# SnowCheetos/CassMantle

Hardware: AMD Instinct MI355X
Metric: SD-1.5 512^2 50-step images/sec (whole node) + p50 guess-score latency (higher is better)
Workload: dtype bf16; 1 GPU; model=sd15 UNet/VAE/CLIP (512x512, 50 steps pndm, cfg 7.5), global_batch=4, seq_len=4096, parallelism=dp1 (rooms)

## Files before the change

### cassmantle_amd/models/layers.py

```python
from __future__ import annotations

import math
import os
from typing import Optional

import torch
import torch.nn as nn

from .. import ops


def _param(shape, std, gen: Optional[torch.Generator], dtype) -> nn.Parameter:
    t = torch.randn(*shape, generator=gen, dtype=torch.float32) * std
    return nn.Parameter(t.to(dtype), requires_grad=False)


def _zeros(shape, dtype) -> nn.Parameter:
    return nn.Parameter(torch.zeros(*shape, dtype=dtype), requires_grad=False)


def _ones(shape, dtype) -> nn.Parameter:
    return nn.Parameter(torch.ones(*shape, dtype=dtype), requires_grad=False)


_GN_FUSE = os.environ.get("CASSMANTLE_GN_FUSE", "1") != "0"
_UP2 = os.environ.get("CASSMANTLE_UP2", "1") != "0"


class StatsArena:

    def __init__(self) -> None:
        self._bufs: dict = {}
        self._need: dict = {}
        self.key = None
        self.buf: Optional[torch.Tensor] = None
        self.off = 0
        self.on = False

    def begin(self, key, x: torch.Tensor) -> "StatsArena":
        self.on = x.device.type == "cuda" and ops.get_mode() == "hip" and _GN_FUSE
        self.key, self.off = key, 0
        if not self.on:
            return self
        self.buf = self._bufs.get(key)
        need = self._need.get(key, 0)
        if need and self.buf is None:
            self.buf = self._bufs[key] = torch.empty(need, device=x.device, dtype=torch.int64)
        if self.buf is not None:
            ops.zero_(self.buf)
        self.device = x.device
        return self

    def take_rows(self, rows: int) -> Optional[torch.Tensor]:
        s = self.take(1, rows)
        return None if s is None else s.view(rows, 2)

    def take(self, B: int, C: int) -> Optional[torch.Tensor]:
        if not self.on:
            return None
        n = B * C * 2
        end = self.off + n
        if self.buf is not None and end <= self.buf.numel():
            s = self.buf[self.off:end].view(B, C, 2)
        else:
            self._need[self.key] = max(self._need.get(self.key, 0), end)
            s = ops.new_stats(B, C, self.device)
        self.off = end
        return s


class Linear(nn.Module):
    def __init__(self, fin: int, fout: int, bias: bool = True, gen=None, dtype=torch.bfloat16,
                 std: Optional[float] = None):
        super().__init__()
        self.fin, self.fout = fin, fout
        self.weight = _param((fout, fin), std if std is not None else 1.0 / math.sqrt(fin), gen, dtype)
        self.bias = _param((fout,), 0.02, gen, dtype) if bias else None

    def forward(self, x, residual=None, act=None, stats=None, row_stats=None):
        return ops.linear(x, self.weight, self.bias, residual=residual, act=act, stats=stats, row_stats=row_stats)


class Conv2d(nn.Module):

    def __init__(self, cin: int, cout: int, k: int = 3, stride: int = 1, padding: Optional[int] = None,
                 bias: bool = True, gen=None, dtype=torch.bfloat16):
        super().__init__()
        self.cin, self.cout, self.k, self.stride = cin, cout, k, stride
        self.padding = (k // 2) if padding is None else padding
        self.weight = _param((cout, k, k, cin), 1.0 / math.sqrt(cin * k * k), gen, dtype)
        self.bias = _param((cout,), 0.02, gen, dtype) if bias else None

    upsampling = False
    pad_in = 0

    def _derived(self, name: str, key, fn):
        buf = self._buffers.get(name)
        if buf is None or getattr(self, "_key_" + name, None) != key or buf.device != self.weight.device:
            self.register_buffer(name, fn(), persistent=False)
            setattr(self, "_key_" + name, key)
        return self._buffers[name]

    def up2_weights(self):
        return self._derived("w4", self.weight._version, lambda: ops.fold_upsample_weights(self.weight))

    def padded_weight(self, cin: int):
        return self._derived("wpad", (self.weight._version, cin),
                             lambda: torch.nn.functional.pad(self.weight, (0, cin - self.cin)).contiguous())

    def prepare(self) -> None:
        if self.upsampling and self.k == 3 and self.cin % 64 == 0:
            self.up2_weights()
        if self.pad_in > self.cin:
            self.padded_weight(self.pad_in)

    def forward(self, x, residual=None, upsample=False, chan_bias=None, stats=None, out=None):
        if out is not None:
            w = self.padded_weight(x.shape[-1]) if x.shape[-1] > self.cin else self.weight
            return ops.conv2d(x, w, self.bias, self.stride, self.padding, residual=residual,
                              upsample=upsample, chan_bias=chan_bias, stats=stats, out=out)
        if x.shape[-1] > self.cin:
            return ops.conv2d(x, self.padded_weight(x.shape[-1]), self.bias, self.stride, self.padding,
                              residual=residual, upsample=upsample, chan_bias=chan_bias, stats=stats)
        if upsample and self.k == 3 and self.stride == 1 and _UP2 and x.device.type == "cuda" \
                and ops.get_mode() == "hip" and self.cin % 64 == 0:
            return ops.conv2d_up2(x, self.weight, self.up2_weights(), self.bias, residual=residual,
                                  chan_bias=chan_bias, stats=stats)
        if self.k == 1 and self.stride == 1 and not upsample and chan_bias is None:
            return ops.linear(x, self.weight.view(self.cout, self.cin), self.bias, residual=residual, stats=stats)
        return ops.conv2d(x, self.weight, self.bias, self.stride, self.padding, residual=residual,
                          upsample=upsample, chan_bias=chan_bias, stats=stats)


class GroupNorm(nn.Module):
    def __init__(self, groups: int, channels: int, eps: float = 1e-5, dtype=torch.bfloat16):
        super().__init__()
        self.groups, self.eps = groups, eps
        self.weight = _ones((channels,), dtype)
        self.bias = _zeros((channels,), dtype)

    def forward(self, x, silu=False, stats=None, stats2=None):
        return ops.group_norm(x, self.groups, self.weight, self.bias, self.eps, silu, stats=stats, stats2=stats2)


class LayerNorm(nn.Module):
    def __init__(self, dim: int, eps: float = 1e-5, dtype=torch.bfloat16):
        super().__init__()
        self.eps = eps
        self.weight = _ones((dim,), dtype)
        self.bias = _zeros((dim,), dtype)

    def forward(self, x):
        return ops.layer_norm(x, self.weight, self.bias, self.eps)


class SelfAttention(nn.Module):

    def __init__(self, dim: int, heads: int, gen=None, dtype=torch.bfloat16, qkv_bias=False,
                 out_bias=True):
        super().__init__()
        self.dim, self.heads = dim, heads
        self.head_dim = dim // heads
        self.to_qkv = Linear(dim, 3 * dim, bias=qkv_bias, gen=gen, dtype=dtype)
        self.to_out = Linear(dim, dim, bias=out_bias, gen=gen, dtype=dtype)

    def forward(self, x, residual=None, causal=False, kv_lens=None, fp8=False, qkv=None, kv8=None,
                row_stats=None):
        if qkv is None:
            qkv = self.to_qkv(x)
        B, N = qkv.shape[0], qkv.shape[1]
        C = self.dim
        qkv = qkv.view(B, N, 3, self.heads, self.head_dim)
        if kv8 is not None:
            assert fp8 and kv_lens is None, "kv8: fp8 self-attention without key lengths"
            o = ops.attention(qkv[:, :, 0], qkv[:, :, 1], qkv[:, :, 2], causal=causal, fp8=True, kv8=kv8)
        else:
            o = ops.attention(qkv[:, :, 0], qkv[:, :, 1], qkv[:, :, 2], causal=causal, kv_lens=kv_lens, fp8=fp8)
        return self.to_out(o.reshape(B, N, C), residual=residual, row_stats=row_stats)


class CrossAttention(nn.Module):
    def __init__(self, dim: int, ctx_dim: int, heads: int, gen=None, dtype=torch.bfloat16):
        super().__init__()
        self.dim, self.heads = dim, heads
        self.head_dim = dim // heads
        self.to_q = Linear(dim, dim, bias=False, gen=gen, dtype=dtype)
        self.to_kv = Linear(ctx_dim, 2 * dim, bias=False, gen=gen, dtype=dtype)
        self.to_out = Linear(dim, dim, bias=True, gen=gen, dtype=dtype)

    _kv = None
    _kv8 = None

    def forward(self, x, ctx, residual=None, fp8=False, q=None, row_stats=None):
        if q is None:
            q = self.to_q(x)
        B, N = q.shape[0], q.shape[1]
        C = self.dim
        q = q.view(B, N, self.heads, self.head_dim)
        kv8 = None
        if self._kv is not None and self._kv.shape[0] == B:
            kv = self._kv.view(B, self._kv.shape[1], 2, self.heads, self.head_dim)
            kv8 = self._kv8 if fp8 else None
        else:
            kv = self.to_kv(ctx).view(B, ctx.shape[1], 2, self.heads, self.head_dim)
        o = ops.attention(q, kv[:, :, 0], kv[:, :, 1], fp8=fp8, kv8=kv8)
        return self.to_out(o.reshape(B, N, C), residual=residual, row_stats=row_stats)


class GEGLUFeedForward(nn.Module):
    def __init__(self, dim: int, mult: int = 4, gen=None, dtype=torch.bfloat16):
        super().__init__()
        inner = dim * mult
        self.proj_in = Linear(dim, 2 * inner, gen=gen, dtype=dtype)
        self.proj_out = Linear(inner, dim, gen=gen, dtype=dtype)

    def forward(self, x, residual=None):
        return self.proj_out(self.proj_in(x, act="geglu"), residual=residual)
```

### cassmantle_amd/models/unet.py

```python
from __future__ import annotations

import os
from dataclasses import dataclass, field
from typing import List, Optional, Sequence, Tuple

import torch
import torch.nn as nn

from .. import ops
from .layers import (Conv2d, CrossAttention, GEGLUFeedForward, GroupNorm, LayerNorm, Linear,
                     SelfAttention, StatsArena)


@dataclass
class UNetConfig:
    in_channels: int = 4
    out_channels: int = 4
    block_out_channels: Tuple[int, ...] = (320, 640, 1280, 1280)
    down_attn: Tuple[bool, ...] = (True, True, True, False)
    transformer_depth: Tuple[int, ...] = (1, 1, 1, 1)
    mid_transformer_depth: int = 1
    layers_per_block: int = 2
    heads: Tuple[int, ...] = (8, 8, 8, 8)
    head_dim: Optional[int] = None
    cross_attention_dim: int = 768
    norm_groups: int = 32
    norm_eps: float = 1e-5
    transformer_norm_eps: float = 1e-6
    time_proj_dim: int = 320
    time_embed_dim: int = 1280
    linear_projection: bool = False
    addition_embed: bool = False
    addition_time_embed_dim: int = 256
    projection_class_embeddings_input_dim: int = 2816
    sample_size: int = 64

    def level_heads(self, i: int) -> int:
        if self.head_dim is not None:
            return self.block_out_channels[i] // self.head_dim
        return self.heads[i]


SD15_UNET = UNetConfig()
SDXL_UNET = UNetConfig(block_out_channels=(320, 640, 1280), down_attn=(False, True, True),
                       transformer_depth=(0, 2, 10), mid_transformer_depth=10, heads=(5, 10, 20),
                       head_dim=64, cross_attention_dim=2048, linear_projection=True,
                       addition_embed=True, sample_size=128)
TINY_UNET = UNetConfig(block_out_channels=(32, 64), down_attn=(True, False), transformer_depth=(1, 1),
                       heads=(2, 2), layers_per_block=1, cross_attention_dim=32, norm_groups=8,
                       time_proj_dim=32, time_embed_dim=64, sample_size=8)


class ResnetBlock(nn.Module):
    def __init__(self, cin: int, cout: int, temb: int, groups: int, eps: float, gen, dtype):
        super().__init__()
        self.norm1 = GroupNorm(groups, cin, eps, dtype)
        self.conv1 = Conv2d(cin, cout, 3, gen=gen, dtype=dtype)
        self.time_emb_proj = Linear(temb, cout, gen=gen, dtype=dtype)
        self.norm2 = GroupNorm(groups, cout, eps, dtype)
        self.conv2 = Conv2d(cout, cout, 3, gen=gen, dtype=dtype)
        self.conv_shortcut = Conv2d(cin, cout, 1, padding=0, gen=gen, dtype=dtype) if cin != cout else None

    def forward(self, x, temb_silu, tb_all=None, arena: Optional[StatsArena] = None, xs=None, xs2=None):
        pair = isinstance(x, tuple)
        B = x[0].shape[0] if pair else x.shape[0]
        cout = self.conv1.cout
        if pair:
            g = self.norm1
            h = ops.group_norm_cat(x[0], x[1], g.groups, g.weight, g.bias, g.eps, True, stats=xs, stats2=xs2)
        else:
            h = self.norm1(x, silu=True, stats=xs, stats2=xs2)
        if tb_all is not None:
            tb = tb_all[:, self._tb_off:self._tb_off + self.time_emb_proj.fout]
        else:
            tb = self.time_emb_proj(temb_silu)
        s1 = arena.take(B, cout) if arena is not None else None
        h = self.conv1(h, chan_bias=tb, stats=s1)
        h = self.norm2(h, silu=True, stats=s1)
        if pair and self.conv_shortcut is None:
            sc = torch.cat(x, dim=-1)
        elif pair:
            cs = self.conv_shortcut
            sc = ops.linear_cat(x[0], x[1], cs.weight.view(cs.cout, cs.cin), cs.bias)
        else:
            sc = self.conv_shortcut(x) if self.conv_shortcut is not None else x
        s2 = arena.take(B, cout) if arena is not None else None
        return self.conv2(h, residual=sc, stats=s2), s2


_LN_FOLD = os.environ.get("CASSMANTLE_LN_FOLD", "1") == "1"
_LN_ROWSTATS = os.environ.get("CASSMANTLE_LN_ROWSTATS", "1") == "1"
_GN_FOLD = os.environ.get("CASSMANTLE_GN_FOLD", "1") == "1"
_FF_ROWSTATS = os.environ.get("CASSMANTLE_FF_ROWSTATS", "1") == "1"


def _row_stats_wanted(x: torch.Tensor) -> bool:
    return (_LN_ROWSTATS and x.device.type == "cuda" and ops.get_mode() == "hip" and ops.LN_FOLD_MODE == 1
            and x.shape[-1] not in (320, 640) and x.shape[-1] % 8 == 0 and x.numel() // x.shape[-1] >= 1024)


_FP8_KV_EPILOGUE = os.environ.get("CASSMANTLE_FP8_KV_EPILOGUE", "1") == "1"


class BasicTransformerBlock(nn.Module):
    def __init__(self, dim: int, heads: int, ctx_dim: int, gen, dtype):
        super().__init__()
        self.norm1 = LayerNorm(dim, 1e-5, dtype)
        self.attn1 = SelfAttention(dim, heads, gen=gen, dtype=dtype)
        self.norm2 = LayerNorm(dim, 1e-5, dtype)
        self.attn2 = CrossAttention(dim, ctx_dim, heads, gen=gen, dtype=dtype)
        self.norm3 = LayerNorm(dim, 1e-5, dtype)
        self.ff = GEGLUFeedForward(dim, 4, gen=gen, dtype=dtype)

    _folds = None

    def _fold_sources(self):
        return ((self.norm1, self.attn1.to_qkv), (self.norm2, self.attn2.to_q), (self.norm3, self.ff.proj_in))

    def folds(self):
        key = tuple((n.weight._version, None if n.bias is None else n.bias._version, l.weight._version,
                     None if l.bias is None else l.bias._version) for n, l in self._fold_sources())
        buf = self._buffers.get("fold0_w")
        if buf is None or self._fold_key != key or buf.device != self.norm1.weight.device:
            for i, (n, l) in enumerate(self._fold_sources()):
                for tag, t in zip(("w", "s", "b"), ops.ln_fold(n.weight, n.bias, l.weight, l.bias)):
                    self.register_buffer(f"fold{i}_{tag}", t, persistent=False)
            self._fold_key = key
        return tuple((self._buffers[f"fold{i}_w"], self._buffers[f"fold{i}_s"], self._buffers[f"fold{i}_b"])
                     for i in range(3))

    def forward(self, x, ctx, fp8=False, arena: Optional[StatsArena] = None, xrs=None, out_stats=False):
        if _LN_FOLD and x.device.type == "cuda" and ops.get_mode() == "hip":
            f = self.folds()
            n1, n2, n3 = self.norm1, self.norm2, self.norm3
            want = arena is not None and _row_stats_wanted(x)
            rows = x.numel() // x.shape[-1]
            kv8 = None
            if fp8 and _FP8_KV_EPILOGUE and ops.kv8_ok(x, self.attn1.head_dim):
                kv8 = ops.kv8_image(x.shape[0], x.shape[1], x.shape[2], x.device)
            qkv = ops.ln_linear(x, n1.weight, n1.bias, n1.eps, self.attn1.to_qkv.weight, fold=f[0], kv8=kv8,
                                row_stats=xrs if want else None)
            r2 = arena.take_rows(rows) if want else None
            x = self.attn1(None, residual=x, fp8=fp8, qkv=qkv, kv8=kv8, row_stats=r2)
            q = ops.ln_linear(x, n2.weight, n2.bias, n2.eps, self.attn2.to_q.weight, fold=f[1], row_stats=r2)
            r3 = arena.take_rows(rows) if want else None
            x = self.attn2(None, ctx, residual=x, fp8=fp8, q=q, row_stats=r3)
            h = ops.ln_linear(x, n3.weight, n3.bias, n3.eps, self.ff.proj_in.weight, act="geglu", fold=f[2],
                              row_stats=r3)
            r4 = arena.take_rows(rows) if (want and out_stats and _FF_ROWSTATS) else None
            return self.ff.proj_out(h, residual=x, row_stats=r4), r4
        x = self.attn1(self.norm1(x), residual=x, fp8=fp8)
        x = self.attn2(self.norm2(x), ctx, residual=x, fp8=fp8)
        x = self.ff(self.norm3(x), residual=x)
        return x, None


class Transformer2D(nn.Module):
    def __init__(self, dim: int, heads: int, depth: int, ctx_dim: int, groups: int, gen, dtype):
        super().__init__()
        self.norm = GroupNorm(groups, dim, 1e-6, dtype)
        self.proj_in = Linear(dim, dim, gen=gen, dtype=dtype)
        self.transformer_blocks = nn.ModuleList(
            [BasicTransformerBlock(dim, heads, ctx_dim, gen, dtype) for _ in range(depth)])
        self.proj_out = Linear(dim, dim, gen=gen, dtype=dtype)

    def forward(self, x, ctx, fp8=False, arena: Optional[StatsArena] = None, xs=None):
        B, H, W, C = x.shape
        hrs = None
        if (_GN_FOLD and xs is not None and C == 320 and (H * W) % 256 == 0 and x.device.type == "cuda"
                and ops.get_mode() == "hip"):
            n = self.norm
            h = ops.gn_linear(x.view(B, H * W, C), xs, n.weight, n.bias, n.groups, n.eps, self.proj_in.weight,
                              self.proj_in.bias)
        else:
            h = self.norm(x, stats=xs).view(B, H * W, C)
            hrs = arena.take_rows(B * H * W) if (arena is not None and _LN_FOLD and _row_stats_wanted(h)) else None
            h = self.proj_in(h, row_stats=hrs)
        rs = hrs
        nblk = len(self.transformer_blocks)
        for i, blk in enumerate(self.transformer_blocks):
            h, rs = blk(h, ctx, fp8=fp8, arena=arena, xrs=rs, out_stats=i + 1 < nblk)
        so = arena.take(B, C) if arena is not None else None
        return self.proj_out(h, residual=x.view(B, H * W, C), stats=so).view(B, H, W, C), so


class Downsample(nn.Module):
    def __init__(self, c: int, gen, dtype):
        super().__init__()
        self.conv = Conv2d(c, c, 3, stride=2, padding=1, gen=gen, dtype=dtype)

    def forward(self, x, arena: Optional[StatsArena] = None):
        so = arena.take(x.shape[0], self.conv.cout) if arena is not None else None
        return self.conv(x, stats=so), so


class Upsample(nn.Module):
    def __init__(self, c: int, gen, dtype):
        super().__init__()
        self.conv = Conv2d(c, c, 3, gen=gen, dtype=dtype)
        self.conv.upsampling = True

    def forward(self, x, arena: Optional[StatsArena] = None):
        so = arena.take(x.shape[0], self.conv.cout) if arena is not None else None
        return self.conv(x, upsample=True, stats=so), so


class UNet(nn.Module):
    def __init__(self, cfg: UNetConfig = SD15_UNET, seed: int = 0, dtype=torch.bfloat16):
        super().__init__()
        self.cfg = cfg
        gen = torch.Generator().manual_seed(seed)
        ch = cfg.block_out_channels
        g, eps, te = cfg.norm_groups, cfg.norm_eps, cfg.time_embed_dim
        self.conv_in = Conv2d(cfg.in_channels, ch[0], 3, gen=gen, dtype=dtype)
        self.conv_in.pad_in = 8 if cfg.in_channels % 8 else 0
        self.time_linear_1 = Linear(cfg.time_proj_dim, te, gen=gen, dtype=dtype)
        self.time_linear_2 = Linear(te, te, gen=gen, dtype=dtype)
        if cfg.addition_embed:
            self.add_linear_1 = Linear(cfg.projection_class_embeddings_input_dim, te, gen=gen, dtype=dtype)
            self.add_linear_2 = Linear(te, te, gen=gen, dtype=dtype)
        self.down = nn.ModuleList()
        skip_ch: List[int] = [ch[0]]
        cur = ch[0]
        n = len(ch)
        for i in range(n):
            blk = nn.Module()
            blk.resnets = nn.ModuleList()
            blk.attentions = nn.ModuleList()
            for j in range(cfg.layers_per_block):
                blk.resnets.append(ResnetBlock(cur, ch[i], te, g, eps, gen, dtype))
                cur = ch[i]
                if cfg.down_attn[i]:
                    blk.attentions.append(Transformer2D(cur, cfg.level_heads(i), cfg.transformer_depth[i],
                                                       cfg.cross_attention_dim, g, gen, dtype))
                skip_ch.append(cur)
            blk.downsampler = Downsample(cur, gen, dtype) if i < n - 1 else None
            if i < n - 1:
                skip_ch.append(cur)
            self.down.append(blk)
        self.mid_res1 = ResnetBlock(cur, cur, te, g, eps, gen, dtype)
        self.mid_attn = Transformer2D(cur, cfg.level_heads(n - 1), cfg.mid_transformer_depth,
                                      cfg.cross_attention_dim, g, gen, dtype)
        self.mid_res2 = ResnetBlock(cur, cur, te, g, eps, gen, dtype)
        self.up = nn.ModuleList()
        rev = list(reversed(range(n)))
# ... 152 lines not shown
```

### cassmantle_amd/ops/__init__.py

```python
from __future__ import annotations

import math
import os
from typing import List, Optional

import torch

from . import reference as ref
from ._ext import ext, ext_available, ext_error

_MODE = os.environ.get("CASSMANTLE_OPS", "hip").lower()


def set_mode(mode: str) -> None:
    global _MODE
    assert mode in ("hip", "torch")
    _MODE = mode


def get_mode() -> str:
    return _MODE


def _use_hip(t: torch.Tensor) -> bool:
    if t.device.type != "cuda":
        return False
    if _MODE == "torch":
        return False
    if not ext_available():
        raise RuntimeError(
            "cassmantle_amd HIP extension is not loaded on a GPU device "
            f"({ext_error()}); run `python -m cassmantle_amd.build` or set CASSMANTLE_OPS=torch "
            "explicitly for the stock-PyTorch baseline")
    return True


_TUNE_PATH = os.path.join(os.path.dirname(os.path.abspath(__file__)), "gemm_tuning.json")
_RECORD: Optional[list] = None
_tune_loaded = False
_DIAG_TWICE = os.environ.get("CASSMANTLE_DIAG_TWICE", "0") == "1"
if _DIAG_TWICE and os.environ.get("CASSMANTLE_DIAG_TWICE_ACK") != "wrong-results":
    raise RuntimeError("CASSMANTLE_DIAG_TWICE=1 makes every GEMM / conv result WRONG (epilogue "
                       "statistics and residuals applied twice); it is a timing diagnostic for "
                       "tools/diag_twice.py only: also set CASSMANTLE_DIAG_TWICE_ACK=wrong-results")


def load_gemm_tuning(path: Optional[str] = None) -> int:
    global _tune_loaded
    if os.environ.get("CASSMANTLE_GEMM_TUNE", "1") == "0" or not ext_available():
        return 0
    if _tune_loaded and path is None:
        return ext().gemm_tune_size()
    import json
    p = path or os.environ.get("CASSMANTLE_GEMM_TUNE_PATH") or _TUNE_PATH
    _tune_loaded = True
    if not os.path.exists(p):
        return 0
    with open(p) as f:
        data = json.load(f)
    for e in data.get("entries", []):
        ext().gemm_tune_set(e["key"], int(e["cfg"]), int(e["split"]))
    return ext().gemm_tune_size()


def record_gemms(on: bool) -> Optional[list]:
    global _RECORD
    if on:
        _RECORD = []
        ext().gemm_record_keys(True)
        return _RECORD
    rec, _RECORD = _RECORD, None
    ext().gemm_record_keys(False)
    return rec


_PF_SERIAL = os.environ.get("CASSMANTLE_PF_SERIAL", "0") == "1"


def _launch(fn, *args, **kw):
    if not _tune_loaded:
        load_gemm_tuning()
    if _PF_SERIAL:
        prefetch(args[2] if fn is ext().gemm_cat else args[1])
    if _DIAG_TWICE:
        fn(*args, **kw)
    fn(*args, **kw)
    if _RECORD is not None:
        call = lambda: fn(*args, **kw)
        call.fn, call.args, call.kw = fn, args, kw
        _RECORD.append((ext().gemm_last_key(), call))


_ACT = {None: 0, "none": 0, "gelu": 1, "silu": 2, "quick_gelu": 3, "geglu": 4, "gelu_tanh": 5, "swiglu": 6}


STAT_SCALE = (2.0 ** 24, 2.0 ** 16)


def h2d(t: torch.Tensor, device) -> torch.Tensor:
    device = torch.device(device)
    if device.type != "cuda":
        return t.to(device)
    return t.pin_memory().to(device, non_blocking=True)


def new_stats(B: int, C: int, device) -> torch.Tensor:
    return zero_(torch.empty((B, C, 2), device=device, dtype=torch.int64))


def stats_to_float(stats: torch.Tensor) -> torch.Tensor:
    sc = torch.tensor([1.0 / STAT_SCALE[0], 1.0 / STAT_SCALE[1]], dtype=torch.float64, device=stats.device)
    return stats.double() * sc


def channel_stats_ref(y: torch.Tensor, stats: torch.Tensor) -> None:
    B, C = y.shape[0], y.shape[-1]
    yf = y.reshape(B, -1, C).double()
    stats[..., 0] += torch.round(yf.sum(1) * STAT_SCALE[0]).to(torch.int64)
    stats[..., 1] += torch.round((yf * yf).sum(1) * STAT_SCALE[1]).to(torch.int64)


def channel_stats(y: torch.Tensor, stats: torch.Tensor) -> None:
    if _use_hip(y):
        ext().channel_stats(y.contiguous(), stats)
    else:
        channel_stats_ref(y, stats)


def linear(x: torch.Tensor, w: torch.Tensor, bias: Optional[torch.Tensor] = None,
           residual: Optional[torch.Tensor] = None, act: Optional[str] = None,
           stats: Optional[torch.Tensor] = None, out: Optional[torch.Tensor] = None,
           row_stats: Optional[torch.Tensor] = None) -> torch.Tensor:
    if not _use_hip(x):
        if x.device.type == "cuda":
            y = _torch_linear(x, w, bias, residual, act)
        else:
            y = ref.linear(x, w, bias, residual, act)
        if stats is not None:
            channel_stats_ref(y, stats)
        return y if out is None else out.copy_(y)
    K = x.shape[-1]
    x2 = x.reshape(-1, K)
    if not x2.is_contiguous():
        x2 = x2.contiguous()
    N = w.shape[0] // 2 if act in ("geglu", "swiglu") else w.shape[0]
    if out is None:
        out = torch.empty((x2.shape[0], N), device=x.device, dtype=x.dtype)
    else:
        assert out.is_contiguous() and out.dtype == x.dtype and out.numel() == x2.shape[0] * N, "linear: bad out"
    o2 = out.view(x2.shape[0], N)
    r2 = residual.reshape(-1, N) if residual is not None else None
    hw = x2.shape[0] // x.shape[0] if stats is not None else 0
    if row_stats is not None:
        _launch(ext().gemm, x2, w, bias, r2, o2, _ACT[act], stats, hw, row_stats=row_stats)
    else:
        _launch(ext().gemm, x2, w, bias, r2, o2, _ACT[act], stats, hw)
    return out.view(*x.shape[:-1], N)


def gn_linear(x: torch.Tensor, stats: torch.Tensor, gamma: torch.Tensor, beta: torch.Tensor, groups: int,
              eps: float, w: torch.Tensor, bias: Optional[torch.Tensor] = None,
              residual: Optional[torch.Tensor] = None) -> torch.Tensor:
    B, C = x.shape[0], x.shape[-1]
    if not _use_hip(x):
        xn = group_norm(x, groups, gamma, beta, eps, False, stats=stats)
        return linear(xn, w, bias, residual=residual)
    rows = x.numel() // C
    x2 = x.reshape(rows, C)
    if not x2.is_contiguous():
        x2 = x2.contiguous()
    N = w.shape[0]
    out = torch.empty((rows, N), device=x.device, dtype=x.dtype)
    r2 = residual.reshape(rows, N) if residual is not None else None
    _launch(ext().gemm, x2, w, bias, r2, out, 0, None, 0, gn_stats=stats, gn_gamma=gamma, gn_beta=beta,
            gn_groups=int(groups), gn_hw=rows // B, gn_eps=float(eps))
    return out.reshape(*x.shape[:-1], N)


def ln_fold(ln_weight: torch.Tensor, ln_bias: Optional[torch.Tensor], w: torch.Tensor,
            bias: Optional[torch.Tensor] = None):
    wf = (w.float() * ln_weight.float()[None, :]).to(w.dtype).contiguous()
    wsum = wf.float().sum(1).contiguous()
    b = torch.zeros(w.shape[0], device=w.device, dtype=torch.float32)
    if ln_bias is not None:
        b = b + w.float() @ ln_bias.float()
    if bias is not None:
        b = b + bias.float()
    return wf, wsum, b.to(w.dtype).contiguous()


def row_stats(x: torch.Tensor, eps: float) -> torch.Tensor:
    if not _use_hip(x):
        xf = x.float().reshape(-1, x.shape[-1])
        mean = xf.mean(-1)
        var = xf.var(-1, unbiased=False)
        return torch.stack([mean, (var + eps).rsqrt()], dim=-1)
    out = torch.empty((x.numel() // x.shape[-1], 2), device=x.device, dtype=torch.float32)
    ext().row_stats(x.contiguous(), out, float(eps))
    return out


LN_FOLD_MODE = int(os.environ.get("CASSMANTLE_LN_FOLD_MODE", "1"))


def ln_linear(x: torch.Tensor, ln_weight: torch.Tensor, ln_bias: Optional[torch.Tensor], eps: float,
              w: torch.Tensor, bias: Optional[torch.Tensor] = None, residual: Optional[torch.Tensor] = None,
              act: Optional[str] = None, fold=None, kv8: Optional[torch.Tensor] = None,
              row_stats: Optional[torch.Tensor] = None) -> torch.Tensor:
    K = x.shape[-1]
    rows = x.numel() // K
    if fold is None or not _use_hip(x) or rows <= 8 or K % 8 or (LN_FOLD_MODE == 2 and K not in (320, 640)):
        y = linear(layer_norm(x, ln_weight, ln_bias, eps), w, bias, residual=residual, act=act)
        if kv8 is not None:
            _pack_qkv8(y, kv8)
        return y
    wf, wsum, bf = fold
    x2 = x.reshape(rows, K)
    if not x2.is_contiguous():
        x2 = x2.contiguous()
    N = wf.shape[0] // 2 if act in ("geglu", "swiglu") else wf.shape[0]
    out = torch.empty((rows, N), device=x.device, dtype=x.dtype)
    r2 = residual.reshape(rows, N) if residual is not None else None
    fx = {"ln_rows_fx": row_stats} if row_stats is not None else {}
    if kv8 is not None:
        C = N // 3
        _launch(ext().gemm, x2, wf, bf, r2, out, _ACT[act], None, 0, None, wsum, float(eps), kv8, C,
                int(x.shape[-2]), C // 64, **fx)
    elif fx:
        _launch(ext().gemm, x2, wf, bf, r2, out, _ACT[act], None, 0, None, wsum, float(eps), **fx)
    else:
        _launch(ext().gemm, x2, wf, bf, r2, out, _ACT[act], None, 0, None, wsum, float(eps))
    return out.reshape(*x.shape[:-1], N)


def kv8_image(B: int, N: int, C: int, device) -> torch.Tensor:
    return torch.empty(2 * B * N * C, device=device, dtype=torch.uint8)


def kv8_ok(x: torch.Tensor, head_dim: int) -> bool:
    return (_use_hip(x) and x.dim() == 3 and head_dim == 64 and x.shape[1] % 64 == 0 and x.shape[-1] % 64 == 0
            and x.shape[-1] not in (320, 640))


def _pack_qkv8(y: torch.Tensor, kv8: torch.Tensor) -> None:
    B, N, C3 = y.shape
    C = C3 // 3
    qkv = y.view(B, N, 3, C // 64, 64)
    pack_kv_fp8(qkv[:, :, 1], qkv[:, :, 2], out=kv8)


def linear_cat(x: torch.Tensor, x2: torch.Tensor, w: torch.Tensor, bias: Optional[torch.Tensor] = None,
               residual: Optional[torch.Tensor] = None, stats: Optional[torch.Tensor] = None) -> torch.Tensor:
    Ca, K = x.shape[-1], x.shape[-1] + x2.shape[-1]
    rows = x.numel() // Ca
    if not _use_hip(x) or Ca % 64 or K % 64 or rows <= 8:
        return linear(torch.cat([x, x2], dim=-1), w, bias, residual=residual, stats=stats)
    N = w.shape[0]
    out = torch.empty((rows, N), device=x.device, dtype=x.dtype)
    r2 = residual.reshape(rows, N) if residual is not None else None
    hw = rows // x.shape[0] if stats is not None else 0
    _launch(ext().gemm_cat, x.reshape(rows, Ca).contiguous(), x2.reshape(rows, K - Ca).contiguous(), w, bias, r2, out,
            stats, hw)
    return out.reshape(*x.shape[:-1], N)


def _torch_linear(x, w, bias, residual, act):
    import torch.nn.functional as F
    y = F.linear(x, w, bias)
    if act == "geglu":
        h, g = y.chunk(2, dim=-1)
        y = h * F.gelu(g)
    elif act == "swiglu":
        h, g = y.chunk(2, dim=-1)
        y = h * F.silu(g)
    elif act == "gelu":
        y = F.gelu(y)
    elif act == "gelu_tanh":
        y = F.gelu(y, approximate="tanh")
    elif act == "silu":
        y = F.silu(y)
    elif act == "quick_gelu":
        y = y * torch.sigmoid(1.702 * y)
    if residual is not None:
        y = y + residual
    return y


def conv2d(x: torch.Tensor, w: torch.Tensor, bias: Optional[torch.Tensor] = None, stride: int = 1,
           padding: int = 1, residual: Optional[torch.Tensor] = None, upsample: bool = False,
           chan_bias: Optional[torch.Tensor] = None, stats: Optional[torch.Tensor] = None,
           out: Optional[torch.Tensor] = None) -> torch.Tensor:
    if not _use_hip(x):
        if x.device.type == "cuda":
            y = _torch_conv(x, w, bias, stride, padding, residual, upsample, chan_bias)
        else:
            y = ref.conv2d(x, w, bias, stride, padding, residual, upsample, chan_bias)
        if stats is not None:
            channel_stats_ref(y, stats)
        return y if out is None else out.copy_(y)
    B, H, W, Cin = x.shape
    Cout, kh, kw, _ = w.shape
    if Cin % 8 != 0:
        pad = 8 - Cin % 8
        x = torch.nn.functional.pad(x, (0, pad))
        w = torch.nn.functional.pad(w, (0, pad))
        Cin += pad
    Hi, Wi = (2 * H, 2 * W) if upsample else (H, W)
    Ho = (Hi + 2 * padding - kh) // stride + 1
    Wo = (Wi + 2 * padding - kw) // stride + 1
    if out is None:
        out = torch.empty((B, Ho, Wo, Cout), device=x.device, dtype=x.dtype)
    else:
        assert out.shape == (B, Ho, Wo, Cout) and out.dtype == x.dtype and out.is_contiguous(), "conv2d: bad out"
    _launch(ext().conv2d, x.contiguous(), w, bias, residual, chan_bias, out, stride, padding, int(upsample), stats)
    return out


_UP2_ROWS = ([[1.0, 0.0, 0.0], [0.0, 1.0, 1.0]], [[1.0, 1.0, 0.0], [0.0, 0.0, 1.0]])


def fold_upsample_weights(w: torch.Tensor) -> torch.Tensor:
    wf = w.float()
    outs = []
    for a in (0, 1):
        ra = torch.tensor(_UP2_ROWS[a], device=w.device)
        for b in (0, 1):
            rb = torch.tensor(_UP2_ROWS[b], device=w.device)
            outs.append(torch.einsum("tk,sl,oklc->otsc", ra, rb, wf))
    return torch.stack(outs).to(w.dtype).contiguous()


def conv2d_up2(x: torch.Tensor, w: torch.Tensor, w4: Optional[torch.Tensor] = None,
               bias: Optional[torch.Tensor] = None, residual: Optional[torch.Tensor] = None,
               chan_bias: Optional[torch.Tensor] = None, stats: Optional[torch.Tensor] = None) -> torch.Tensor:
    B, H, W, Cin = x.shape
    if not _use_hip(x) or Cin % 64 or w.shape[1] != 3:
        return conv2d(x, w, bias, 1, 1, residual=residual, upsample=True, chan_bias=chan_bias, stats=stats)
    if w4 is None:
        w4 = fold_upsample_weights(w)
    out = torch.empty((B, 2 * H, 2 * W, w.shape[0]), device=x.device, dtype=x.dtype)
    _launch(ext().conv2d_up2, x.contiguous(), w4, bias, residual, chan_bias, out, stats)
    return out


def _torch_conv(x, w, bias, stride, padding, residual, upsample, chan_bias):
    import torch.nn.functional as F
    xi = x.permute(0, 3, 1, 2)
    if upsample:
        xi = F.interpolate(xi, scale_factor=2.0, mode="nearest")
    wi = w.permute(0, 3, 1, 2)
    y = F.conv2d(xi.contiguous(memory_format=torch.channels_last),
                 wi.contiguous(memory_format=torch.channels_last), bias, stride=stride, padding=padding)
    y = y.permute(0, 2, 3, 1)
    if chan_bias is not None:
        y = y + chan_bias[:, None, None, :]
    if residual is not None:
        y = y + residual
    return y.contiguous()


def _group_norm_from_stats_ref(x, num_groups, weight, bias, eps, silu, stats):
    B, C = x.shape[0], x.shape[-1]
    S = x.numel() // (B * C)
    st = stats_to_float(stats).view(B, num_groups, C // num_groups, 2).sum(2)
    n = S * (C // num_groups)
    mean = st[..., 0] / n
    var = (st[..., 1] / n - mean * mean).clamp_min(0)
    rstd = (var + eps).rsqrt()
    cg = C // num_groups
    mean_c = mean.repeat_interleave(cg, 1).float()
    rstd_c = rstd.repeat_interleave(cg, 1).float()
    shape = [B] + [1] * (x.dim() - 2) + [C]
    y = (x.float() - mean_c.view(shape)) * rstd_c.view(shape) * weight.float() + bias.float()
    if silu:
        y = torch.nn.functional.silu(y)
    return y.to(x.dtype)


def group_norm(x: torch.Tensor, num_groups: int, weight: torch.Tensor, bias: torch.Tensor,
               eps: float, silu: bool = False, stats: Optional[torch.Tensor] = None,
               stats2: Optional[torch.Tensor] = None) -> torch.Tensor:
    if stats is not None:
        if not _use_hip(x):
            st = stats if stats2 is None else torch.cat([stats, stats2], dim=1)
            return _group_norm_from_stats_ref(x, num_groups, weight, bias, eps, silu, st)
        out = torch.empty_like(x)
        ext().group_norm_stats(x.contiguous(), stats, stats2, weight, bias, out, num_groups, float(eps), int(silu))
        return out
    if not _use_hip(x):
        if x.device.type == "cuda":
            import torch.nn.functional as F
            B, C = x.shape[0], x.shape[-1]
            xi = x.reshape(B, -1, C).transpose(1, 2)
            y = F.group_norm(xi, num_groups, weight, bias, eps)
            if silu:
                y = F.silu(y)
            return y.transpose(1, 2).reshape(x.shape).contiguous()
        return ref.group_norm(x, num_groups, weight, bias, eps, silu)
    out = torch.empty_like(x)
    ext().group_norm(x.contiguous(), weight, bias, out, num_groups, float(eps), int(silu))
    return out


def group_norm_cat(x: torch.Tensor, x2: torch.Tensor, num_groups: int, weight: torch.Tensor, bias: torch.Tensor,
                   eps: float, silu: bool = False, stats: Optional[torch.Tensor] = None,
                   stats2: Optional[torch.Tensor] = None) -> torch.Tensor:
    if stats is None or stats2 is None or not _use_hip(x) or x.shape[-1] % 8 or x2.shape[-1] % 8:
        return group_norm(torch.cat([x, x2], dim=-1), num_groups, weight, bias, eps, silu, stats=stats, stats2=stats2)
    out = torch.empty((*x.shape[:-1], x.shape[-1] + x2.shape[-1]), device=x.device, dtype=x.dtype)
    ext().group_norm_cat(x.contiguous(), x2.contiguous(), stats, stats2, weight, bias, out, num_groups, float(eps),
                         int(silu))
    return out


def layer_norm(x: torch.Tensor, weight: torch.Tensor, bias: Optional[torch.Tensor], eps: float) -> torch.Tensor:
    if not _use_hip(x):
        if x.device.type == "cuda":
            import torch.nn.functional as F
            return F.layer_norm(x, (x.shape[-1],), weight, bias, eps)
        return ref.layer_norm(x, weight, bias, eps)
    out = torch.empty_like(x)
    ext().layer_norm(x.contiguous(), weight, bias, out, float(eps))
    return out


def embed_layer_norm(word: torch.Tensor, ids: torch.Tensor, pos: torch.Tensor, add: Optional[torch.Tensor],
                     weight: torch.Tensor, bias: Optional[torch.Tensor], eps: float) -> torch.Tensor:
    B, T = ids.shape
    if not _use_hip(word):
        x = word[ids] + pos[:T][None]
        if add is not None:
            x = x + add
        return layer_norm(x, weight, bias, eps)
    out = torch.empty((B, T, word.shape[-1]), device=word.device, dtype=word.dtype)
    ext().embed_layer_norm(word, ids.contiguous().view(-1), pos, T, add, weight, bias, out, float(eps))
    return out


def rms_norm(x: torch.Tensor, weight: torch.Tensor, eps: float) -> torch.Tensor:
    if not _use_hip(x):
        return ref.rms_norm(x, weight, eps)
    out = torch.empty_like(x)
    ext().rms_norm(x.contiguous(), weight, out, float(eps))
    return out


def rms_linear(x: torch.Tensor, gamma: torch.Tensor, eps: float, w: torch.Tensor,
               bias: Optional[torch.Tensor] = None, residual: Optional[torch.Tensor] = None,
               act: Optional[str] = None) -> torch.Tensor:
    K = x.shape[-1]
    rows = x.numel() // K
    if not _use_hip(x) or rows > 8 or K % 8:
        return linear(rms_norm(x, gamma, eps), w, bias, residual=residual, act=act)
    x2 = x.reshape(rows, K)
    if not x2.is_contiguous():
        x2 = x2.contiguous()
    N = w.shape[0] // 2 if act in ("geglu", "swiglu") else w.shape[0]
    out = torch.empty((rows, N), device=x.device, dtype=x.dtype)
    r2 = residual.reshape(rows, N) if residual is not None else None
    ext().gemm_rms(x2, gamma, float(eps), w, bias, r2, out, _ACT[act])
    return out.reshape(*x.shape[:-1], N)


def rope_kv(qkv: torch.Tensor, pos0: torch.Tensor, q_out: torch.Tensor, k_cache: torch.Tensor,
            v_cache: torch.Tensor, heads: int, kv_heads: int, theta: float) -> None:
    if not _use_hip(qkv):
        ref.rope_kv(qkv, pos0, q_out, k_cache, v_cache, heads, kv_heads, theta)
        return
# ... 549 lines not shown
```

### cassmantle_amd/ops/csrc/bindings.cpp

```cpp
#include <torch/extension.h>
#include <atomic>
#include <ATen/hip/HIPContext.h>
#include <c10/hip/HIPStream.h>
#include <hip/hip_ext.h>

#include "gemm_tiles.h"
#include "kernels.h"

namespace {

hipStream_t cur_stream() { return c10::hip::getCurrentHIPStream().stream(); }

#define CHECK_DEV(t) TORCH_CHECK((t).is_cuda(), #t " must be a GPU tensor")
#define CHECK_BF16(t) TORCH_CHECK((t).scalar_type() == at::kBFloat16, #t " must be bf16")
#define CHECK_CONTIG(t) TORCH_CHECK((t).is_contiguous(), #t " must be contiguous")

const uint16_t* bptr(const at::Tensor& t) { return reinterpret_cast<const uint16_t*>(t.data_ptr()); }
uint16_t* bptr_mut(at::Tensor& t) { return reinterpret_cast<uint16_t*>(t.data_ptr()); }
const uint16_t* opt_bptr(const c10::optional<at::Tensor>& t) {
  if (!t.has_value() || !t->defined()) return nullptr;
  CHECK_DEV(*t);
  CHECK_BF16(*t);
  CHECK_CONTIG(*t);
  return bptr(*t);
}

long long* opt_stats(const c10::optional<at::Tensor>& t, long long images, int N) {
  if (!t.has_value() || !t->defined()) return nullptr;
  CHECK_DEV(*t);
  CHECK_CONTIG(*t);
  TORCH_CHECK(t->scalar_type() == at::kLong && t->numel() == images * N * 2,
              "stats must be a zeroed int64 fixed-point [images, N, 2] tensor (ops.new_stats)");
  return reinterpret_cast<long long*>(t->data_ptr<int64_t>());
}

static std::atomic<int> g_raster[2] = {{-1}, {-1}};
static void raster_from_env() {
  static const bool once = [] {
    const char* e = getenv("CASSMANTLE_GEMM_RASTER");
    int a = 0, b = -1;
    if (e != nullptr) {
      if (sscanf(e, "%d,%d", &a, &b) < 2) b = a;
    } else {
      b = 0;
    }
    int expect = -1;
    g_raster[0].compare_exchange_strong(expect, a);
    expect = -1;
    g_raster[1].compare_exchange_strong(expect, b);
    return true;
  }();
  (void)once;
}
void gemm_set_raster(int64_t plain, int64_t gated) {
  raster_from_env();
  g_raster[0].store((int)plain);
  g_raster[1].store((int)gated);
}

void run_gemm(GemmArgs& p, const at::Tensor& like) {
  raster_from_env();
  p.raster = g_raster[(p.act == 4 || p.act == 6) ? 1 : 0].load(std::memory_order_relaxed);
  TORCH_CHECK(p.stats == nullptr || (p.N % 8 == 0 && p.ldc == p.N),
              "gemm/conv2d stats: the output channel count must be a multiple of 8 (GroupNorm consumers)");
  const GemmPlan plan = gemm_plan(p);
  p.cfg = plan.cfg;
  p.split = plan.split;
  if (p.kv8 != nullptr) p.split = 1;
  long long* post_stats = nullptr;
  if (p.stats != nullptr && (p.out_f32 || p.M <= 8 || (p.batch != 1 && !p.parity) || p.act == 4 || p.act == 6)) {
    post_stats = p.stats;
    p.stats = nullptr;
  }
  if (p.split > 1) {
    auto ws = at::empty({(long long)p.split * p.batch * p.M * p.N}, like.options().dtype(at::kFloat));
    launch_gemm(p, ws.data_ptr<float>(), cur_stream());
  } else {
    launch_gemm(p, nullptr, cur_stream());
  }
  if (post_stats != nullptr)
    launch_channel_stats(reinterpret_cast<const uint16_t*>(p.C), post_stats, p.M / p.stats_hw, p.stats_hw, p.N,
                         cur_stream());
}

void gemm(const at::Tensor& x, const at::Tensor& w, const c10::optional<at::Tensor>& bias,
          const c10::optional<at::Tensor>& residual, at::Tensor& out, int64_t act,
          const c10::optional<at::Tensor>& stats, int64_t stats_hw,
          const c10::optional<at::Tensor>& ln_rows, const c10::optional<at::Tensor>& ln_wsum, double ln_eps,
          const c10::optional<at::Tensor>& kv8, int64_t kv8_col0, int64_t kv8_ntok, int64_t kv8_hk,
          const c10::optional<at::Tensor>& ln_rows_fx, const c10::optional<at::Tensor>& row_stats,
          const c10::optional<at::Tensor>& gn_stats, const c10::optional<at::Tensor>& gn_gamma,
          const c10::optional<at::Tensor>& gn_beta, int64_t gn_groups, int64_t gn_hw, double gn_eps) {
  CHECK_DEV(x); CHECK_BF16(x); CHECK_BF16(w); CHECK_CONTIG(w); CHECK_CONTIG(out);
  TORCH_CHECK(x.dim() == 2 && w.dim() == 2 && out.dim() == 2, "gemm: 2-D operands expected");
  TORCH_CHECK(x.stride(1) == 1, "gemm: x rows must be contiguous");
  GemmArgs p;
  p.A = bptr(x); p.W = bptr(w); p.bias = opt_bptr(bias); p.residual = opt_bptr(residual);
  p.M = (int)x.size(0); p.K = (int)x.size(1); p.N = (int)out.size(1); p.Nw = (int)w.size(0);
  p.lda = (int)x.stride(0); p.ldc = p.N; p.act = (int)act;
  TORCH_CHECK(w.size(1) == p.K, "gemm: K mismatch");
  TORCH_CHECK(out.size(0) == p.M, "gemm: M mismatch");
  if (act == 4 || act == 6) {
    TORCH_CHECK(p.Nw == 2 * p.N && p.K % 8 == 0 && p.N % 4 == 0, "geglu/swiglu: W must be [2N,K], K%8==0, N%4==0");
  } else {
    TORCH_CHECK(p.Nw == p.N, "gemm: N mismatch");
  }
  if (residual.has_value() && residual->defined()) TORCH_CHECK(residual->numel() == out.numel(), "gemm: residual shape");
  if (out.scalar_type() == at::kFloat) {
    p.out_f32 = 1;
  } else {
    CHECK_BF16(out);
  }
  p.C = out.data_ptr();
  if (kv8.has_value() && kv8->defined()) {
    CHECK_DEV(*kv8); CHECK_CONTIG(*kv8);
    TORCH_CHECK(kv8->scalar_type() == at::kByte && kv8_ntok > 0 && kv8_ntok % 64 == 0 && p.M % kv8_ntok == 0 &&
                    kv8_hk > 0 && kv8_col0 % 8 == 0 && kv8_col0 + 128 * kv8_hk == p.N && act == 0 &&
                    !p.out_f32 && !(residual.has_value() && residual->defined()) && !(stats.has_value() && stats->defined()),
                "gemm kv8: uint8 image, 64-aligned tokens per image, K|V heads ending the output, plain epilogue");
    TORCH_CHECK(kv8->numel() == 2LL * p.M * kv8_hk * 64, "gemm kv8: image size");
    p.kv8 = kv8->data_ptr<uint8_t>();
    p.kv8_col0 = (int)kv8_col0; p.kv8_ntok = (int)kv8_ntok; p.kv8_hk = (int)kv8_hk;
  }
  if (stats.has_value() && stats->defined()) {
    TORCH_CHECK(stats_hw > 0 && p.M % stats_hw == 0, "gemm: stats_hw must divide the rows");
    p.stats_hw = (int)stats_hw;
    p.stats = opt_stats(stats, p.M / stats_hw, p.N);
  }
  if (gn_stats.has_value() && gn_stats->defined()) {
    TORCH_CHECK(gn_gamma.has_value() && gn_beta.has_value() && gn_groups > 0 && gn_hw > 0 && p.M % gn_hw == 0,
                "gemm: gn_stats needs gamma, beta, groups and rows per image");
    CHECK_DEV(*gn_stats); CHECK_CONTIG(*gn_stats);
    TORCH_CHECK(gn_stats->scalar_type() == at::kLong && gn_stats->numel() == 2LL * (p.M / gn_hw) * p.K,
                "gemm: gn_stats int64 [images, K, 2]");
    TORCH_CHECK(!(ln_wsum.has_value() && ln_wsum->defined()) && !(row_stats.has_value() && row_stats->defined()) &&
                    !(kv8.has_value() && kv8->defined()) && !(stats.has_value() && stats->defined()),
                "gemm: gn_stats excludes LayerNorm folds, row / GroupNorm output statistics and kv8");
    p.gn_stats = reinterpret_cast<const long long*>(gn_stats->data_ptr<int64_t>());
    p.gn_gamma = opt_bptr(gn_gamma);
    p.gn_beta = opt_bptr(gn_beta);
    p.gn_groups = (int)gn_groups;
    p.gn_hw = (int)gn_hw;
    p.gn_eps = (float)gn_eps;
    if (gemm_areg_ok(p)) {
      run_gemm(p, out);
      return;
    }
    TORCH_CHECK(x.is_contiguous() && p.K % 8 == 0 && p.K % gn_groups == 0, "gemm gn fallback: contiguous rows");
    at::Tensor xn = at::empty_like(x);
    launch_group_norm_cs(bptr(x), nullptr, p.gn_stats, p.K, nullptr, p.gn_gamma, p.gn_beta, bptr_mut(xn),
                         p.M / gn_hw, gn_hw, p.K, (int)gn_groups, (float)gn_eps, 0, cur_stream());
    p.gn_stats = nullptr; p.gn_gamma = nullptr; p.gn_beta = nullptr;
    p.A = bptr(xn);
    run_gemm(p, out);
    return;
  }
  if (row_stats.has_value() && row_stats->defined()) {
    CHECK_DEV(*row_stats); CHECK_CONTIG(*row_stats);
    TORCH_CHECK(row_stats->scalar_type() == at::kLong && row_stats->numel() == 2LL * p.M,
                "gemm: row_stats zeroed int64 [M, 2]");
    TORCH_CHECK(p.stats == nullptr && p.kv8 == nullptr && !p.out_f32 && p.batch == 1 && p.M > 8 && p.N % 8 == 0 &&
                    p.ldc % 8 == 0 && p.K % 8 == 0 && p.lda % 8 == 0,
                "gemm: row_stats needs the LDS-staged bf16 epilogue (no GroupNorm stats / kv8, N % 8 == 0, M > 8)");
    p.row_stats = reinterpret_cast<long long*>(row_stats->data_ptr<int64_t>());
  }
  if (ln_rows_fx.has_value() && ln_rows_fx->defined()) {
    TORCH_CHECK(ln_wsum.has_value() && ln_wsum->defined() && ln_eps > 0 && !(ln_rows.has_value() && ln_rows->defined()),
                "gemm: ln_rows_fx needs ln_wsum and ln_eps, and excludes ln_rows");
    CHECK_DEV(*ln_rows_fx); CHECK_CONTIG(*ln_rows_fx); CHECK_DEV(*ln_wsum); CHECK_CONTIG(*ln_wsum);
    TORCH_CHECK(ln_rows_fx->scalar_type() == at::kLong && ln_rows_fx->numel() == 2LL * p.M, "gemm: ln_rows_fx int64 [M, 2]");
    TORCH_CHECK(ln_wsum->scalar_type() == at::kFloat && ln_wsum->numel() == p.Nw, "gemm: ln_wsum fp32 [Nw]");
    TORCH_CHECK(p.M > 8 && p.K % 8 == 0 && p.lda % 8 == 0 && !p.out_f32, "gemm: folded LayerNorm needs the MFMA path");
    p.ln_rows_fx = reinterpret_cast<const long long*>(ln_rows_fx->data_ptr<int64_t>());
    p.ln_wsum = ln_wsum->data_ptr<float>();
    p.ln_eps = (float)ln_eps;
    run_gemm(p, out);
    return;
  }
  if (ln_rows.has_value() && ln_rows->defined()) {
    TORCH_CHECK(ln_wsum.has_value() && ln_wsum->defined(), "gemm: ln_rows needs ln_wsum");
    CHECK_DEV(*ln_rows); CHECK_CONTIG(*ln_rows); CHECK_DEV(*ln_wsum); CHECK_CONTIG(*ln_wsum);
    TORCH_CHECK(ln_rows->scalar_type() == at::kFloat && ln_rows->numel() == 2LL * p.M, "gemm: ln_rows fp32 [M, 2]");
    TORCH_CHECK(ln_wsum->scalar_type() == at::kFloat && ln_wsum->numel() == p.Nw, "gemm: ln_wsum fp32 [Nw]");
    TORCH_CHECK(p.M > 8 && p.K % 8 == 0 && p.lda % 8 == 0, "gemm: folded LayerNorm needs the MFMA path (M > 8)");
    TORCH_CHECK(!p.out_f32 || p.act == 0, "gemm: folded LayerNorm with fp32 output supports no activation");
    p.ln_rows = ln_rows->data_ptr<float>();
    p.ln_wsum = ln_wsum->data_ptr<float>();
  } else if (ln_wsum.has_value() && ln_wsum->defined() && ln_eps > 0) {
    CHECK_DEV(*ln_wsum); CHECK_CONTIG(*ln_wsum);
    TORCH_CHECK(ln_wsum->scalar_type() == at::kFloat && ln_wsum->numel() == p.Nw, "gemm: ln_wsum fp32 [Nw]");
    TORCH_CHECK(p.M > 8 && p.K % 8 == 0 && p.lda % 8 == 0 && !p.out_f32, "gemm: folded LayerNorm needs the MFMA path");
    p.ln_wsum = ln_wsum->data_ptr<float>();
    p.ln_eps = (float)ln_eps;
    static const bool inkernel = [] { const char* e = getenv("CASSMANTLE_LN_INKERNEL"); return !(e && e[0] == '0'); }();
    if (!inkernel || !gemm_areg_ok(p)) {
      TORCH_CHECK(x.is_contiguous() && p.K <= 4096, "gemm: folded LayerNorm row statistics need contiguous rows");
      at::Tensor rows = at::empty({p.M, 2}, x.options().dtype(at::kFloat));
      launch_row_stats(bptr(x), rows.data_ptr<float>(), p.M, p.K, (float)ln_eps, cur_stream());
      p.ln_rows = rows.data_ptr<float>();
      p.ln_eps = 0.f;
      run_gemm(p, out);
      return;
    }
  }
  run_gemm(p, out);
}

void row_stats(const at::Tensor& x, at::Tensor& out, double eps) {
  CHECK_DEV(x); CHECK_BF16(x); CHECK_CONTIG(x); CHECK_CONTIG(out);
  const int D = (int)x.size(-1);
  TORCH_CHECK(D % 8 == 0 && D <= 4096, "row_stats: D % 8 == 0 and D <= 4096");
  TORCH_CHECK(out.scalar_type() == at::kFloat && out.numel() == 2 * (x.numel() / D), "row_stats: out fp32 [rows, 2]");
  launch_row_stats(bptr(x), out.data_ptr<float>(), x.numel() / D, D, (float)eps, cur_stream());
}

void gemm_cat(const at::Tensor& x, const at::Tensor& x2, const at::Tensor& w, const c10::optional<at::Tensor>& bias,
              const c10::optional<at::Tensor>& residual, at::Tensor& out, const c10::optional<at::Tensor>& stats,
              int64_t stats_hw) {
  CHECK_DEV(x); CHECK_BF16(x); CHECK_CONTIG(x); CHECK_BF16(x2); CHECK_CONTIG(x2); CHECK_BF16(w); CHECK_CONTIG(w);
  CHECK_BF16(out); CHECK_CONTIG(out);
  TORCH_CHECK(x.dim() == 2 && x2.dim() == 2 && w.dim() == 2 && out.dim() == 2 && x.size(0) == x2.size(0),
              "gemm_cat: 2-D operands with equal rows expected");
  GemmArgs p;
  p.A = bptr(x); p.A2 = bptr(x2); p.W = bptr(w); p.bias = opt_bptr(bias); p.residual = opt_bptr(residual);
  p.M = (int)x.size(0); p.ka = (int)x.size(1); p.K = p.ka + (int)x2.size(1);
  p.N = (int)out.size(1); p.Nw = (int)w.size(0);
  p.lda = p.ka; p.lda2 = (int)x2.size(1); p.ldc = p.N;
  TORCH_CHECK(w.size(1) == p.K && p.Nw == p.N && out.size(0) == p.M, "gemm_cat: shape mismatch");
  TORCH_CHECK(p.ka % 64 == 0 && p.K % 64 == 0 && p.M > 8, "gemm_cat: Ca and K must be multiples of 64, M > 8");
  const long long lim = (1LL << 31) - 1;
  TORCH_CHECK(x.numel() * 2 <= lim && x2.numel() * 2 <= lim && w.numel() * 2 <= lim, "gemm_cat: operand too large");
  if (residual.has_value() && residual->defined()) TORCH_CHECK(residual->numel() == out.numel(), "gemm_cat: residual shape");
  p.C = out.data_ptr();
  if (stats.has_value() && stats->defined()) {
    TORCH_CHECK(stats_hw > 0 && p.M % stats_hw == 0, "gemm_cat: stats_hw must divide the rows");
    p.stats_hw = (int)stats_hw;
    p.stats = opt_stats(stats, p.M / stats_hw, p.N);
  }
  run_gemm(p, out);
}

void gemm_rms(const at::Tensor& x, const at::Tensor& gamma, double eps, const at::Tensor& w,
              const c10::optional<at::Tensor>& bias, const c10::optional<at::Tensor>& residual, at::Tensor& out,
              int64_t act) {
  CHECK_DEV(x); CHECK_BF16(x); CHECK_BF16(gamma); CHECK_CONTIG(gamma); CHECK_BF16(w); CHECK_CONTIG(w);
  CHECK_CONTIG(out);
  TORCH_CHECK(x.dim() == 2 && x.stride(1) == 1 && x.size(0) <= 8, "gemm_rms: x [<=8, K] rows contiguous");
  GemmArgs p;
  p.A = bptr(x); p.W = bptr(w); p.bias = opt_bptr(bias); p.residual = opt_bptr(residual);
  p.M = (int)x.size(0); p.K = (int)x.size(1); p.N = (int)out.size(1); p.Nw = (int)w.size(0);
  p.lda = (int)x.stride(0); p.ldc = p.N; p.act = (int)act;
  p.rms_gamma = bptr(gamma); p.rms_eps = (float)eps;
  TORCH_CHECK(gamma.numel() == p.K && w.size(1) == p.K, "gemm_rms: K mismatch");
  TORCH_CHECK(p.Nw == ((act == 4 || act == 6) ? 2 * p.N : p.N), "gemm_rms: N mismatch");
  if (out.scalar_type() == at::kFloat) p.out_f32 = 1;
  else CHECK_BF16(out);
  p.C = out.data_ptr();
  TORCH_CHECK(launch_gemv(p, cur_stream()), "gemm_rms: shape not supported by the GEMV path (K % 8)");
}

void conv2d(const at::Tensor& x, const at::Tensor& w, const c10::optional<at::Tensor>& bias,
            const c10::optional<at::Tensor>& residual, const c10::optional<at::Tensor>& chan_bias, at::Tensor& out,
            int64_t stride, int64_t pad, int64_t upsample, const c10::optional<at::Tensor>& stats) {
  CHECK_DEV(x); CHECK_BF16(x); CHECK_CONTIG(x); CHECK_BF16(w); CHECK_CONTIG(w); CHECK_CONTIG(out); CHECK_BF16(out);
  TORCH_CHECK(x.dim() == 4 && w.dim() == 4 && out.dim() == 4, "conv2d: NHWC 4-D tensors expected");
  GemmArgs p;
  p.conv = 1;
  p.A = bptr(x); p.W = bptr(w); p.bias = opt_bptr(bias); p.residual = opt_bptr(residual);
  if (chan_bias.has_value() && chan_bias->defined()) {
    CHECK_DEV(*chan_bias);
    CHECK_BF16(*chan_bias);
    TORCH_CHECK(chan_bias->dim() == 2 && chan_bias->stride(1) == 1, "conv2d: chan_bias must be [B, Cout] rows");
    p.chan_bias = bptr(*chan_bias);
    p.ldcb = (int)chan_bias->stride(0);
  }
  p.IH = (int)x.size(1); p.IW = (int)x.size(2); p.Cin = (int)x.size(3);
  p.ksize = (int)w.size(1);
  TORCH_CHECK(w.size(2) == p.ksize && w.size(3) == p.Cin, "conv2d: weight must be [Cout,k,k,Cin]");
  p.Ho = (int)out.size(1); p.Wo = (int)out.size(2);
  p.N = (int)out.size(3); p.Nw = (int)w.size(0);
  TORCH_CHECK(p.Nw == p.N && out.size(0) == x.size(0), "conv2d: shape mismatch");
  p.M = (int)(x.size(0) * p.Ho * p.Wo);
  p.K = p.ksize * p.ksize * p.Cin;
  p.lda = p.Cin; p.ldc = p.N;
  p.stride = (int)stride; p.pad = (int)pad; p.upsample = (int)upsample;
  if (residual.has_value() && residual->defined()) TORCH_CHECK(residual->numel() == out.numel(), "conv2d: residual shape");
  if (chan_bias.has_value() && chan_bias->defined())
    TORCH_CHECK(chan_bias->size(0) == x.size(0) && chan_bias->size(1) == p.N, "conv2d: chan_bias must be [B, Cout]");
  p.C = out.data_ptr();
  p.stats_hw = p.Ho * p.Wo;
  p.stats = opt_stats(stats, x.size(0), p.N);
  run_gemm(p, out);
}

void conv2d_up2(const at::Tensor& x, const at::Tensor& w4, const c10::optional<at::Tensor>& bias,
                const c10::optional<at::Tensor>& residual, const c10::optional<at::Tensor>& chan_bias, at::Tensor& out,
                const c10::optional<at::Tensor>& stats) {
  CHECK_DEV(x); CHECK_BF16(x); CHECK_CONTIG(x); CHECK_BF16(w4); CHECK_CONTIG(w4); CHECK_CONTIG(out); CHECK_BF16(out);
  TORCH_CHECK(x.dim() == 4 && w4.dim() == 5 && w4.size(0) == 4 && w4.size(2) == 2 && w4.size(3) == 2 &&
              w4.size(4) == x.size(3), "conv2d_up2: x [B,H,W,Cin], w4 [4,Cout,2,2,Cin]");
  TORCH_CHECK(out.dim() == 4 && out.size(0) == x.size(0) && out.size(1) == 2 * x.size(1) &&
              out.size(2) == 2 * x.size(2) && out.size(3) == w4.size(1), "conv2d_up2: out [B,2H,2W,Cout]");
  GemmArgs p;
  p.conv = 1;
  p.parity = 1;
  p.A = bptr(x); p.W = bptr(w4); p.bias = opt_bptr(bias); p.residual = opt_bptr(residual);
  if (chan_bias.has_value() && chan_bias->defined()) {
    CHECK_DEV(*chan_bias);
    CHECK_BF16(*chan_bias);
    TORCH_CHECK(chan_bias->dim() == 2 && chan_bias->stride(1) == 1 && chan_bias->size(0) == x.size(0) &&
                chan_bias->size(1) == out.size(3), "conv2d_up2: chan_bias must be [B, Cout] rows");
    p.chan_bias = bptr(*chan_bias);
    p.ldcb = (int)chan_bias->stride(0);
  }
  p.IH = (int)x.size(1); p.IW = (int)x.size(2); p.Cin = (int)x.size(3);
  p.ksize = 2; p.stride = 1; p.pad = 1; p.upsample = 0;
  p.Ho = p.IH; p.Wo = p.IW;
  p.N = (int)out.size(3); p.Nw = p.N;
  p.M = (int)(x.size(0) * p.Ho * p.Wo);
  p.K = 4 * p.Cin;
  p.lda = p.Cin; p.ldc = p.N;
  p.batch = 4;
  p.sA = 0; p.sW = (long long)p.N * 4 * p.Cin; p.sC = 0;
  TORCH_CHECK(p.Cin % 64 == 0, "conv2d_up2: Cin % 64 == 0 (buffer-DMA conv path)");
  if (residual.has_value() && residual->defined()) TORCH_CHECK(residual->numel() == out.numel(), "conv2d_up2: residual shape");
  p.C = out.data_ptr();
  p.stats_hw = p.Ho * p.Wo;
  p.stats = opt_stats(stats, x.size(0), p.N);
  run_gemm(p, out);
}

void bmm_nt(const at::Tensor& a, const at::Tensor& b, at::Tensor& out, double alpha) {
  CHECK_DEV(a); CHECK_BF16(a); CHECK_BF16(b); CHECK_CONTIG(out);
  TORCH_CHECK(a.dim() == 3 && b.dim() == 3 && out.dim() == 3, "bmm_nt: 3-D operands");
  TORCH_CHECK(a.stride(2) == 1 && b.stride(2) == 1, "bmm_nt: K must be contiguous");
  GemmArgs p;
  p.A = bptr(a); p.W = bptr(b);
  p.batch = (int)a.size(0);
  p.M = (int)a.size(1); p.K = (int)a.size(2); p.N = (int)b.size(1); p.Nw = p.N;
  p.lda = (int)a.stride(1); p.ldw = (int)b.stride(1); p.sA = a.stride(0); p.sW = b.stride(0);
  p.ldc = p.N; p.sC = (long long)p.M * p.N;
  p.alpha = (float)alpha;
  if (out.scalar_type() == at::kFloat) {
    p.out_f32 = 1;
  } else {
    CHECK_BF16(out);
  }
  p.C = out.data_ptr();
  run_gemm(p, out);
}

void group_norm(const at::Tensor& x, const at::Tensor& gamma, const at::Tensor& beta, at::Tensor& out,
                int64_t groups, double eps, int64_t silu) {
  CHECK_DEV(x); CHECK_BF16(x); CHECK_CONTIG(x); CHECK_BF16(gamma); CHECK_BF16(beta); CHECK_CONTIG(out);
  const int B = (int)x.size(0);
  const int C = (int)x.size(-1);
  const long long S = x.numel() / ((long long)B * C);
  TORCH_CHECK(C % 8 == 0 && C % groups == 0, "group_norm: C must be a multiple of 8 and of groups");
  auto ws = at::empty({group_norm_workspace(B, S, C)}, x.options().dtype(at::kFloat));
  launch_group_norm(bptr(x), bptr(gamma), bptr(beta), bptr_mut(out), ws.data_ptr<float>(), B, S, C, (int)groups,
                    (float)eps, (int)silu, cur_stream());
}

void group_norm_stats(const at::Tensor& x, const at::Tensor& stats_a, const c10::optional<at::Tensor>& stats_b,
                      const at::Tensor& gamma, const at::Tensor& beta, at::Tensor& out, int64_t groups, double eps,
                      int64_t silu) {
  CHECK_DEV(x); CHECK_BF16(x); CHECK_CONTIG(x); CHECK_BF16(gamma); CHECK_BF16(beta); CHECK_CONTIG(out);
  const int B = (int)x.size(0);
  const int C = (int)x.size(-1);
  const long long S = x.numel() / ((long long)B * C);
  TORCH_CHECK(C % 8 == 0 && C % groups == 0, "group_norm_stats: C must be a multiple of 8 and of groups");
  TORCH_CHECK(stats_a.scalar_type() == at::kLong && stats_a.is_contiguous() && stats_a.dim() == 3 &&
              stats_a.size(0) == B && stats_a.size(2) == 2, "group_norm_stats: stats_a must be int64 [B, Ca, 2]");
  const int Ca = (int)stats_a.size(1);
  const long long* sb = nullptr;
  if (stats_b.has_value() && stats_b->defined()) {
    TORCH_CHECK(stats_b->scalar_type() == at::kLong && stats_b->is_contiguous() && stats_b->dim() == 3 &&
                stats_b->size(0) == B && stats_b->size(1) == C - Ca && stats_b->size(2) == 2,
                "group_norm_stats: stats_b must be int64 [B, C - Ca, 2]");
    sb = reinterpret_cast<const long long*>(stats_b->data_ptr<int64_t>());
  } else {
    TORCH_CHECK(Ca == C, "group_norm_stats: stats_a must cover every channel");
  }
  launch_group_norm_cs(bptr(x), nullptr, reinterpret_cast<const long long*>(stats_a.data_ptr<int64_t>()), Ca, sb, bptr(gamma), bptr(beta), bptr_mut(out), B, S, C,
                       (int)groups, (float)eps, (int)silu, cur_stream());
}

void group_norm_cat(const at::Tensor& x, const at::Tensor& x2, const at::Tensor& stats_a, const at::Tensor& stats_b,
                    const at::Tensor& gamma, const at::Tensor& beta, at::Tensor& out, int64_t groups, double eps,
                    int64_t silu) {
  CHECK_DEV(x); CHECK_BF16(x); CHECK_CONTIG(x); CHECK_BF16(x2); CHECK_CONTIG(x2); CHECK_BF16(gamma); CHECK_BF16(beta);
  CHECK_CONTIG(out); CHECK_BF16(out);
  const int B = (int)x.size(0);
  const int Ca = (int)x.size(-1), Cb = (int)x2.size(-1), C = Ca + Cb;
  const long long S = x.numel() / ((long long)B * Ca);
  TORCH_CHECK(x2.size(0) == B && x2.numel() == (long long)B * S * Cb && out.numel() == (long long)B * S * C &&
              out.size(-1) == C, "group_norm_cat: shapes must agree on batch and pixels");
  TORCH_CHECK(Ca % 8 == 0 && Cb % 8 == 0 && C % groups == 0, "group_norm_cat: channel counts");
  TORCH_CHECK(stats_a.scalar_type() == at::kLong && stats_a.is_contiguous() && stats_a.numel() == (long long)B * Ca * 2 &&
              stats_b.scalar_type() == at::kLong && stats_b.is_contiguous() && stats_b.numel() == (long long)B * Cb * 2,
              "group_norm_cat: int64 [B, C, 2] statistics of both inputs expected");
  launch_group_norm_cs(bptr(x), bptr(x2), reinterpret_cast<const long long*>(stats_a.data_ptr<int64_t>()), Ca, reinterpret_cast<const long long*>(stats_b.data_ptr<int64_t>()), bptr(gamma),
                       bptr(beta), bptr_mut(out), B, S, C, (int)groups, (float)eps, (int)silu, cur_stream());
}

void channel_stats(const at::Tensor& x, at::Tensor& stats) {
  CHECK_DEV(x); CHECK_BF16(x); CHECK_CONTIG(x);
  const int B = (int)x.size(0);
  const int C = (int)x.size(-1);
  const long long S = x.numel() / ((long long)B * C);
  TORCH_CHECK(C % 8 == 0, "channel_stats: C % 8 == 0");
  launch_channel_stats(bptr(x), opt_stats(stats, B, C), B, S, C, cur_stream());
}

void layer_norm(const at::Tensor& x, const at::Tensor& gamma, const c10::optional<at::Tensor>& beta, at::Tensor& out,
                double eps) {
  CHECK_DEV(x); CHECK_BF16(x); CHECK_CONTIG(x); CHECK_BF16(gamma); CHECK_CONTIG(out);
  const int D = (int)x.size(-1);
  TORCH_CHECK(D % 8 == 0 && D <= 4096, "layer_norm: D % 8 == 0 and D <= 4096");
  launch_layer_norm(bptr(x), bptr(gamma), opt_bptr(beta), bptr_mut(out), x.numel() / D, D, (float)eps, cur_stream());
}

void embed_layer_norm(const at::Tensor& word, const at::Tensor& ids, const at::Tensor& pos, int64_t seq,
                      const c10::optional<at::Tensor>& add, const at::Tensor& gamma,
                      const c10::optional<at::Tensor>& beta, at::Tensor& out, double eps) {
  CHECK_DEV(word); CHECK_BF16(word); CHECK_CONTIG(word); CHECK_DEV(ids); CHECK_CONTIG(ids);
  CHECK_BF16(pos); CHECK_CONTIG(pos); CHECK_BF16(gamma); CHECK_BF16(out); CHECK_CONTIG(out);
  TORCH_CHECK(ids.scalar_type() == at::kLong, "embed_layer_norm: int64 ids");
  const int D = (int)word.size(-1);
  TORCH_CHECK(D % 8 == 0 && D <= 4096 && pos.size(-1) == D && out.numel() == ids.numel() * D,
              "embed_layer_norm: D % 8 == 0, D <= 4096, out [rows, D]");
  TORCH_CHECK(seq > 0 && pos.size(0) >= seq, "embed_layer_norm: position table shorter than seq");
  launch_embed_layer_norm(bptr(word), reinterpret_cast<const long long*>(ids.data_ptr<int64_t>()), bptr(pos), (int)seq,
                          opt_bptr(add), bptr(gamma), opt_bptr(beta), bptr_mut(out), ids.numel(), D, (float)eps,
                          cur_stream());
}

static AttnArgs attn_args(const at::Tensor& q, const at::Tensor& k, const at::Tensor& v, at::Tensor& out, double scale,
                          int64_t causal, const c10::optional<at::Tensor>& kv_lens) {
  CHECK_DEV(q); CHECK_BF16(q); CHECK_BF16(k); CHECK_BF16(v); CHECK_BF16(out);
  TORCH_CHECK(q.dim() == 4 && k.dim() == 4 && v.dim() == 4 && out.dim() == 4, "attention: [B,N,H,d] tensors");
  TORCH_CHECK(q.stride(3) == 1 && k.stride(3) == 1 && v.stride(3) == 1 && out.stride(3) == 1,
              "attention: head dim must be contiguous");
  AttnArgs a;
  a.q = bptr(q); a.k = bptr(k); a.v = bptr(v); a.o = bptr_mut(out);
// ... 415 lines not shown
  TORCH_CHECK(H > 0 && W > 0 && H < 65536 && W < 65536, "jpeg: image sides must be in 1..65535");
  TORCH_CHECK(out.scalar_type() == at::kByte && out.dim() == 4 && out.size(0) > 0 && out.size(1) == H &&
              out.size(2) == W && out.size(3) == 3, "jpeg: out uint8 [B, H, W, 3]");
  JpegArgs a;
  a.B = (int)out.size(0); a.H = (int)H; a.W = (int)W;
  const int mcu = s420 ? 16 : 8;
  a.nb = s420 ? 6 : 3;
  a.mx = (a.W + mcu - 1) / mcu; a.my = (a.H + mcu - 1) / mcu;
  const long long mcus = (long long)a.B * a.mx * a.my;
  TORCH_CHECK(coef.scalar_type() == at::kShort && coef.numel() == mcus * a.nb * 64,
              "jpeg: coef int16 [B, mcus, blocks, 64]");
  TORCH_CHECK(planes.scalar_type() == at::kByte && planes.numel() == mcus * a.nb * 64,
              "jpeg: planes uint8 [B * mcus * blocks * 64]");
  TORCH_CHECK((double)a.B * a.H * ((a.W + 3) / 4) < 256.0 * 2147483647.0, "jpeg: batch too large for one launch");
  a.qtab = tables.data_ptr<int>();
  a.coef = coef.data_ptr<int16_t>();
  a.planes = planes.data_ptr<uint8_t>();
  a.dec = out.data_ptr<uint8_t>();
  TORCH_CHECK(reinterpret_cast<uintptr_t>(a.planes) % 4 == 0 && reinterpret_cast<uintptr_t>(a.dec) % 4 == 0 &&
              reinterpret_cast<uintptr_t>(a.coef) % 4 == 0, "jpeg: buffers must be 4-byte aligned");
  launch_jpeg_reconstruct(a, cur_stream());
}

void jpeg_entropy_decode(const at::Tensor& staged, int64_t nbytes, const at::Tensor& tables, at::Tensor& buf,
                         int64_t B, int64_t H, int64_t W, int64_t s420, int64_t restart) {
  CHECK_DEV(staged); CHECK_CONTIG(staged); CHECK_DEV(tables); CHECK_CONTIG(tables); CHECK_DEV(buf); CHECK_CONTIG(buf);
  TORCH_CHECK(B > 0 && H > 0 && W > 0 && H < 65536 && W < 65536, "jpeg: image sides must be in 1..65535");
  TORCH_CHECK(restart >= 0 && restart < 65536, "jpeg: restart interval 0..65535");
  TORCH_CHECK(tables.scalar_type() == at::kInt && tables.numel() == 128 + 544 + 1024,
              "jpeg: decode tables int32 [672 + 1024]");
  JpegArgs a;
  a.B = (int)B; a.H = (int)H; a.W = (int)W;
  const int mcu = s420 ? 16 : 8;
  a.nb = s420 ? 6 : 3;
  a.mx = (a.W + mcu - 1) / mcu; a.my = (a.H + mcu - 1) / mcu;
  const long long mcus = (long long)a.mx * a.my;
  a.restart = restart ? (int)restart : (int)mcus;
  a.nint = (int)((mcus + a.restart - 1) / a.restart);
  const long long nivals = B * a.nint, ncoef = B * mcus * a.nb * 64;
  TORCH_CHECK(nivals < 2147483647LL, "jpeg: too many restart intervals for one launch");
  TORCH_CHECK(buf.scalar_type() == at::kShort && buf.numel() == ncoef + 8, "jpeg: buf int16 [B * mcus * blocks * 64 + 8]");
  TORCH_CHECK(nbytes >= 0 && nbytes < 4294967295LL && staged.scalar_type() == at::kByte &&
              staged.numel() >= 8 * nivals + nbytes, "jpeg: staged uint8 [8 * B * intervals + nbytes]");
  TORCH_CHECK(reinterpret_cast<uintptr_t>(staged.data_ptr()) % 4 == 0 && reinterpret_cast<uintptr_t>(buf.data_ptr()) % 16 == 0,
              "jpeg: staged 4-byte aligned, buf 16-byte aligned");
  a.coef = buf.data_ptr<int16_t>();
  JpegDecodeIn d;
  d.intervals = reinterpret_cast<const uint32_t*>(staged.data_ptr<uint8_t>());
  d.bytes = staged.data_ptr<uint8_t>() + 8 * nivals;
  d.nbytes = (uint32_t)nbytes;
  d.tables = reinterpret_cast<const uint32_t*>(tables.data_ptr<int>()) + 128 + 544;
  d.status = reinterpret_cast<unsigned long long*>(a.coef + ncoef);
  d.zero_bytes = (ncoef + 8) * 2;
  launch_jpeg_entropy_decode(a, d, cur_stream());
}

void jpeg_entropy_decode_chunked(const at::Tensor& staged, int64_t nbytes, const at::Tensor& tables, at::Tensor& buf,
                                 int64_t B, int64_t H, int64_t W, int64_t s420, int64_t restart, int64_t extra,
                                 int64_t ngroups, int64_t chunk, int64_t threads) {
  CHECK_DEV(staged); CHECK_CONTIG(staged); CHECK_DEV(tables); CHECK_CONTIG(tables); CHECK_DEV(buf); CHECK_CONTIG(buf);
  TORCH_CHECK(B > 0 && H > 0 && W > 0 && H < 65536 && W < 65536, "jpeg: image sides must be in 1..65535");
  TORCH_CHECK(restart >= 0 && restart < 65536, "jpeg: restart interval 0..65535");
  TORCH_CHECK(tables.scalar_type() == at::kInt && tables.numel() == 128 + 544 + 1024,
              "jpeg: decode tables int32 [672 + 1024]");
  JpegArgs a;
  a.B = (int)B; a.H = (int)H; a.W = (int)W;
  const int mcu = s420 ? 16 : 8;
  a.nb = s420 ? 6 : 3;
  a.mx = (a.W + mcu - 1) / mcu; a.my = (a.H + mcu - 1) / mcu;
  const long long mcus = (long long)a.mx * a.my;
  a.restart = restart ? (int)restart : (int)mcus;
  a.nint = (int)((mcus + a.restart - 1) / a.restart);
  const long long nivals = B * a.nint, ncoef = B * mcus * a.nb * 64;
  TORCH_CHECK(nivals < 2147483647LL && ncoef / 64 < 256LL * 2147483647LL, "jpeg: too many restart intervals or blocks for one launch");
  TORCH_CHECK(buf.scalar_type() == at::kShort && buf.numel() == ncoef + 16, "jpeg: buf int16 [B * mcus * blocks * 64 + 16]");
  TORCH_CHECK(chunk >= 16 && chunk % 16 == 0 && chunk < (1LL << 28), "jpeg: chunk bytes a multiple of 16");
  TORCH_CHECK(threads >= 64 && threads <= 1024 && threads % 64 == 0, "jpeg: 64..1024 lanes per workgroup");
  TORCH_CHECK(ngroups >= 0 && ngroups <= nivals, "jpeg: at most one group per interval");
  TORCH_CHECK(nbytes >= 0 && nbytes < 4294967295LL && staged.scalar_type() == at::kByte && extra % 4 == 0 &&
              extra >= 8 * nivals + nbytes && staged.numel() >= extra + 4 * nivals + 8 * ngroups,
              "jpeg: staged uint8 [8 * B * intervals + nbytes | 4 * B * intervals + 8 * groups]");
  TORCH_CHECK(reinterpret_cast<uintptr_t>(staged.data_ptr()) % 4 == 0 && reinterpret_cast<uintptr_t>(buf.data_ptr()) % 16 == 0,
              "jpeg: staged 4-byte aligned, buf 16-byte aligned");
  a.coef = buf.data_ptr<int16_t>();
  JpegDecodeIn d;
  d.intervals = reinterpret_cast<const uint32_t*>(staged.data_ptr<uint8_t>());
  d.bytes = staged.data_ptr<uint8_t>() + 8 * nivals;
  d.nbytes = (uint32_t)nbytes;
  d.tables = reinterpret_cast<const uint32_t*>(tables.data_ptr<int>()) + 128 + 544;
  d.status = reinterpret_cast<unsigned long long*>(a.coef + ncoef);
  d.zero_bytes = (ncoef + 16) * 2;
  JpegSyncIn y;
  y.lane0 = reinterpret_cast<const uint32_t*>(staged.data_ptr<uint8_t>() + extra);
  y.groups = y.lane0 + nivals;
  y.ngroups = (int)ngroups;
  y.cb = (uint32_t)chunk;
  y.words = reinterpret_cast<uint32_t*>(a.coef + ncoef + 4);
  launch_jpeg_entropy_decode_chunked(a, d, y, (int)threads, cur_stream());
}

void blur_pil_check(const at::Tensor& img, const at::Tensor& out) {
  CHECK_DEV(img); CHECK_CONTIG(img); CHECK_DEV(out); CHECK_CONTIG(out);
  TORCH_CHECK(img.scalar_type() == at::kByte && img.dim() == 3 && img.size(2) == 3 && img.numel() > 0,
              "blur_pil: img uint8 [H, W, 3]");
  TORCH_CHECK(img.size(0) < 65536 && img.size(1) < 65536, "blur_pil: image sides must be below 65536");
  TORCH_CHECK(out.scalar_type() == at::kByte && out.dim() == 4 && out.size(0) > 0 && out.size(1) == img.size(0) &&
              out.size(2) == img.size(1) && out.size(3) == 3, "blur_pil: out uint8 [N, H, W, 3]");
  TORCH_CHECK(out.device() == img.device(), "blur_pil: img and out on one device");
  const char* i0 = static_cast<const char*>(img.data_ptr());
  const char* o0 = static_cast<const char*>(out.data_ptr());
  TORCH_CHECK(i0 + img.numel() <= o0 || o0 + out.numel() <= i0, "blur_pil: out overlaps img");
}

void blur_pil_tiled(const at::Tensor& img, const at::Tensor& table, at::Tensor& out, int64_t rmax) {
  blur_pil_check(img, out);
  CHECK_DEV(table); CHECK_CONTIG(table);
  TORCH_CHECK(table.scalar_type() == at::kInt && table.dim() == 2 && table.size(1) == 4 && table.size(0) > 0 &&
              table.size(0) < 65536 && table.device() == img.device(), "blur_pil: table int32 [n, 4], n < 65536");
  TORCH_CHECK(rmax >= 0 && rmax <= blur_pil_max_tiled_radius(), "blur_pil: the tiled kernel covers box radius <= ",
              blur_pil_max_tiled_radius());
  launch_blur_pil_tiled(img.data_ptr<uint8_t>(), (int)img.size(0), (int)img.size(1), table.data_ptr<int>(),
                        (int)table.size(0), (int)rmax, (int)out.size(0), out.data_ptr<uint8_t>(), cur_stream());
}

void blur_pil_general(const at::Tensor& img, at::Tensor& out, int64_t slot, at::Tensor& scratch, int64_t r,
                      int64_t ww, int64_t fw) {
  blur_pil_check(img, out);
  blur_pil_check(img, scratch);
  TORCH_CHECK(scratch.size(0) == 2, "blur_pil: scratch uint8 [2, H, W, 3]");
  TORCH_CHECK(slot >= 0 && slot < out.size(0), "blur_pil: slot outside out");
  const int64_t one = (int64_t)1 << 24;
  TORCH_CHECK(r >= 0 && r < 32768 && ww >= 0 && fw >= 0 && (2 * r + 1) * ww + 2 * fw <= one,
              "blur_pil: box weights must sum to at most 2^24");
  const char* s0 = static_cast<const char*>(scratch.data_ptr());
  const char* o0 = static_cast<const char*>(out.data_ptr());
  TORCH_CHECK(s0 + scratch.numel() <= o0 || o0 + out.numel() <= s0, "blur_pil: scratch overlaps out");
  const int64_t n = img.numel();
  uint8_t* sp = scratch.data_ptr<uint8_t>();
  launch_blur_pil_general(img.data_ptr<uint8_t>(), (int)img.size(0), (int)img.size(1), (int)r, (uint32_t)ww,
                          (uint32_t)fw, sp, sp + n, out.data_ptr<uint8_t>() + slot * n, cur_stream());
}

}

using nogil = py::call_guard<py::gil_scoped_release>;

PYBIND11_MODULE(_C, m) {
  m.doc() = "cassmantle_amd gfx950 (CDNA4) HIP kernel library";
  m.def("gemm", &gemm, py::arg("x"), py::arg("w"), py::arg("bias"), py::arg("residual"), py::arg("out"),
        py::arg("act"), py::arg("stats"), py::arg("stats_hw"), py::arg("ln_rows") = py::none(),
        py::arg("ln_wsum") = py::none(), py::arg("ln_eps") = 0.0, py::arg("kv8") = py::none(),
        py::arg("kv8_col0") = 0, py::arg("kv8_ntok") = 0, py::arg("kv8_hk") = 0, py::arg("ln_rows_fx") = py::none(),
        py::arg("row_stats") = py::none(), py::arg("gn_stats") = py::none(), py::arg("gn_gamma") = py::none(),
        py::arg("gn_beta") = py::none(), py::arg("gn_groups") = 0, py::arg("gn_hw") = 0, py::arg("gn_eps") = 0.0, nogil());
  m.def("row_stats", &row_stats, nogil());
  m.def("gemm_cat", &gemm_cat, nogil());
  m.def("group_norm_cat", &group_norm_cat, nogil());
  m.def("gemm_tile_menu", []() {
    static const char* const fam[] = {"static", "pingpong", "deep", "areg"};
    py::list rows;
    for (const GemmTile& t : kGemmTiles)
      rows.append(py::make_tuple(t.id, fam[t.family], t.BM, t.BN, std::to_string(t.WM) + "x" + std::to_string(t.WN), t.stages,
                                 t.producers, t.gated()));
    return rows;
  });
  m.def("gemm_set_override", [](int64_t cfg, int64_t split) { gemm_set_override((int)cfg, (int)split); });
  m.def("gemm_tune_set", [](const std::string& key, int64_t cfg, int64_t split) { gemm_tune_set(key, (int)cfg, (int)split); });
  m.def("gemm_tune_clear", []() { gemm_tune_clear(); });
  m.def("gemm_tune_size", []() { return (int64_t)gemm_tune_size(); });
  m.def("gemm_record_keys", [](bool on) { gemm_record_keys(on); });
  m.def("gemm_last_key", []() { return gemm_last_key(); });
  m.def("gemm_last_plan", []() { int c, sp; gemm_last_plan(&c, &sp); return std::vector<int64_t>{c, sp}; });
  m.def("gemm_rms", &gemm_rms, nogil());
  m.def("conv2d", &conv2d, nogil());
  m.def("conv2d_up2", &conv2d_up2, nogil());
  m.def("bmm_nt", &bmm_nt, nogil());
  m.def("group_norm", &group_norm, nogil());
  m.def("layer_norm", &layer_norm, nogil());
  m.def("embed_layer_norm", &embed_layer_norm, nogil());
  m.def("group_norm_stats", &group_norm_stats, nogil());
  m.def("channel_stats", &channel_stats, nogil());
  m.def("attention", &attention, nogil());
  m.def("attention_fp8_pack", &attention_fp8_pack, nogil());
  m.def("attention_fp8_bytes", &attention_fp8_bytes, nogil());
  m.def("gather_cosine", &gather_cosine, nogil());
  m.def("pair_cosine", &pair_cosine, nogil());
  m.def("cosine_gemv", &cosine_gemv, nogil());
  m.def("cosine_topk", &cosine_topk, nogil());
  m.def("mean_pool_l2", &mean_pool_l2, nogil());
  m.def("gaussian_blur", &gaussian_blur, nogil());
  m.def("blur_pil_tiled", &blur_pil_tiled, nogil());
  m.def("blur_pil_general", &blur_pil_general, nogil());
  m.def("blur_pil_max_tiled_radius", []() { return (int64_t)blur_pil_max_tiled_radius(); });
  m.def("to_uint8", &to_uint8, nogil());
  m.def("jpeg_count", &jpeg_count, nogil());
  m.def("jpeg_write", &jpeg_write, nogil());
  m.def("jpeg_reconstruct", &jpeg_reconstruct, nogil());
  m.def("jpeg_entropy_decode", &jpeg_entropy_decode, nogil());
  m.def("jpeg_entropy_decode_chunked", &jpeg_entropy_decode_chunked, nogil());
  m.def("timestep_embedding", &timestep_embedding, nogil());
  m.def("gather_add", &gather_add, nogil());
  m.def("concat2", &concat2, nogil());
  m.def("silu_", &silu_, nogil());
  m.def("latent_init", &latent_init, nogil());
  m.def("finalize_latents", &finalize_latents, nogil());
  m.def("dcopy", &dcopy, nogil());
  m.def("set_fp8_attn_variant", [](int64_t v) { set_fp8_attn_variant((int)v); });
  m.def("set_attn_d40_variant", [](int64_t v) { set_attn_d40_variant((int)v); });
  m.def("gemm_set_raster", &gemm_set_raster);
  m.def("latent_step", &latent_step, nogil());
  m.def("advance_step", &advance_step, nogil());
  m.def("zero_", &zero_, nogil());
  m.def("prefetch", &prefetch, nogil());
  m.def("lm_sample", &lm_sample, nogil());
  m.def("cu_mask_stream", &cu_mask_stream);
  m.def("cu_count", &cu_count);
  m.def("softmax_rows", &softmax_rows, nogil());
  m.def("rms_norm", &rms_norm, nogil());
  m.def("rope_kv", &rope_kv, nogil());
  m.def("decode_attention", &decode_attention, nogil());
  m.attr("arch") = "gfx950";
}
```

### cassmantle_amd/ops/csrc/gemm.hip

```cpp
#include <stdio.h>
#include <stdlib.h>

#include <atomic>
#include <mutex>
#include <string>
#include <unordered_map>

#include "common.h"
#include "gemm_tiles.h"
#include "kernels.h"

void gemm_c0_buf_launch(const GemmArgs& p, float* ws, hipStream_t s);
void gemm_c0_launch(const GemmArgs& p, float* ws, hipStream_t s);
void gemm_c1_launch(const GemmArgs& p, float* ws, hipStream_t s);
void gemm_c2_buf_launch(const GemmArgs& p, float* ws, hipStream_t s);
void gemm_c2_launch(const GemmArgs& p, float* ws, hipStream_t s);
void gemm_c3_launch(const GemmArgs& p, float* ws, hipStream_t s);
void gemm_pp_c0_launch(const GemmArgs& p, float* ws, hipStream_t s);
void gemm_pp_c2_launch(const GemmArgs& p, float* ws, hipStream_t s);

namespace {

constexpr int BK = 64;

// ... 48 lines not shown
  if (p.chan_bias) o += bf2f(p.chan_bias[(long long)(m / (p.Ho * p.Wo)) * (p.ldcb ? p.ldcb : p.N) + n]);
  o = apply_act(o, p.act);
  if (p.residual) o += bf2f(p.residual[(long long)m * p.ldc + n]);
  if (p.out_f32)
    reinterpret_cast<float*>(p.C)[(long long)batch * p.sC + (long long)m * p.ldc + n] = o;
  else
    reinterpret_cast<uint16_t*>(p.C)[(long long)batch * p.sC + (long long)m * p.ldc + n] = f2bf(o);
}

bool family_runs(GemmTileFamily f, const GemmArgs& p) {
  if (f == kTileStatic) return true;
  if (f == kTileAreg) return gemm_areg_ok(p);
  if (f == kTilePingPong && (p.N % 8 != 0 || p.ldc % 8 != 0 || (p.ldcb ? p.ldcb : p.N) % 4 != 0)) return false;
  return !p.out_f32 && buf_ok(p) && p.K % BK == 0 && (!p.conv || (!p.upsample && p.Cin % 64 == 0)) && p.N > 16;
}

bool cfg_runs(int cfg, const GemmArgs& p) {
  const GemmTile* t = gemm_tile(cfg);
  return t != nullptr && family_runs(t->family, p);
}

std::mutex g_tune_mu;
std::unordered_map<std::string, GemmPlan> g_tune;
thread_local std::string g_last_key;
thread_local GemmPlan g_last_plan{0, 1};
std::atomic<bool> g_record_key{false};

}

std::string gemm_key(const GemmArgs& p) {
  char buf[192];
  snprintf(buf, sizeof(buf), "m%d n%d k%d w%d b%d c%d:%d:%d:%d:%d:%d:%d:%d p%d a%d g%d s%d r%d cb%d ln%d f%d",
           p.M, p.N, p.K, p.Nw, p.batch, p.conv, p.IH, p.IW, p.Cin, p.stride, p.ksize, p.pad, p.upsample, p.parity,
           p.A2 != nullptr, is_gated(p.act) ? 1 : 0, p.stats != nullptr, p.residual != nullptr, p.chan_bias != nullptr,
           (p.ln_rows != nullptr || p.ln_rows_fx != nullptr) ? 1 : (p.ln_wsum != nullptr ? 2 : (p.gn_stats ? 3 : 0)),
           p.out_f32);
  return std::string(buf);
}

void gemm_tune_set(const std::string& key, int cfg, int split) {
  std::lock_guard<std::mutex> g(g_tune_mu);
  g_tune[key] = GemmPlan{cfg, split};
}
void gemm_tune_clear() {
  std::lock_guard<std::mutex> g(g_tune_mu);
  g_tune.clear();
}
int gemm_tune_size() {
  std::lock_guard<std::mutex> g(g_tune_mu);
  return (int)g_tune.size();
}
void gemm_record_keys(bool on) { g_record_key = on; }
std::string gemm_last_key() { return g_last_key; }
void gemm_last_plan(int* cfg, int* split) { *cfg = g_last_plan.cfg; *split = g_last_plan.split; }

static int env_int(const char* name, int dflt) {
  const char* e = getenv(name);
  return e ? atoi(e) : dflt;
}

static std::atomic<int> g_force_cfg{-2}, g_force_split{0};
void gemm_set_override(int cfg, int split) {
  g_force_cfg = cfg;
  g_force_split = split;
}

static GemmPlan gemm_plan_impl(const GemmArgs& p);
GemmPlan gemm_plan(const GemmArgs& p) {
  GemmPlan r = gemm_plan_impl(p);
  if (p.row_stats != nullptr) {
    if (r.cfg == kGemmAregTile) r.cfg = 3;
    r.split = 1;
  }
  g_last_plan = r;
  return r;
}

static GemmPlan gemm_plan_impl(const GemmArgs& p) {
  GemmPlan best{0, 1};
  if (g_force_cfg.load(std::memory_order_acquire) == -2) {
    static const bool from_env = [] {
      g_force_split.store(env_int("CASSMANTLE_GEMM_SPLIT", 0));
      int expect = -2;
      g_force_cfg.compare_exchange_strong(expect, env_int("CASSMANTLE_GEMM_CFG", -1));
      return true;
    }();
    (void)from_env;
  }
  const int force_cfg = g_force_cfg.load(), force_split = g_force_split.load();
  if (g_record_key) g_last_key = gemm_key(p);
  if (p.ln_wsum != nullptr && p.ln_rows == nullptr && p.ln_rows_fx == nullptr) return GemmPlan{kGemmAregTile, 1};
  if (p.gn_stats != nullptr) return GemmPlan{kGemmAregTile, 1};
  if (force_cfg < 0) {
    bool have = false;
    GemmPlan tp{0, 1};
    {
      std::lock_guard<std::mutex> g(g_tune_mu);
      if (!g_tune.empty()) {
        auto it = g_tune.find(gemm_key(p));
        if (it != g_tune.end()) { tp = it->second; have = true; }
      }
    }
    if (have && cfg_runs(tp.cfg, p)) return tp;
  }
  static const int use_big = env_int("CASSMANTLE_GEMM_8WAVE", 0);
  const bool gated = p.act == ACT_GEGLU || p.act == ACT_SWIGLU;
  int only = -1;
  static const int pp_auto = env_int("CASSMANTLE_GEMM_PP", 0);
  const bool pp = pp_auto && family_runs(kTilePingPong, p);
  if (force_cfg >= 0 && cfg_runs(force_cfg, p)) {
    const GemmTile& ft = *gemm_tile(force_cfg);
    if (ft.family == kTileAreg) return GemmPlan{ft.id, 1};
    if ((ft.BN <= 16) == (p.N <= 16)) {
      if (gated) {
        best.cfg = ft.gated() ? ft.id : gemm_default_tile(ft.model ? ft.family : kTileDeep, true);
        return best;
      }
      only = ft.id;
    }
  }
  if (gated) {
    if (pp && (p.N % 64 == 0) && (long long)(p.N / 64) * ((p.M + 255) / 256) >= 256)
      best.cfg = gemm_default_tile(kTilePingPong, true);
    return best;
  }
  const int nk = (p.K + BK - 1) / BK;
  const bool can_split = p.N % 4 == 0 && p.K % 8 == 0 && p.M > 8;
  double best_t = 1e30;
  for (const GemmTile& tc : kGemmTiles) {
    if (only >= 0 ? tc.id != only
                  : !tc.model || (tc.family == kTileStatic && tc.WM * tc.WN == 8 && !use_big) ||
                        (tc.family == kTilePingPong && !pp))
      continue;
    if ((tc.BN <= 16) != (p.N <= 16)) continue;
    const long long tiles = (long long)((p.N + tc.BN - 1) / tc.BN) * ((p.M + tc.BM - 1) / tc.BM) * p.batch;
    const double waste = (double)tc.BN * ((p.N + tc.BN - 1) / tc.BN) / p.N;
    for (int split = 1; split <= GEMM_MAX_SPLIT; ++split) {
      if (split > 1 && (!can_split || nk / split < 4)) break;
      const long long blocks = tiles * split;
      const long long rounds = (blocks + tc.slots - 1) / tc.slots;
      const int kper = (nk + split - 1) / split;
      const double tile_cost = (0.55 + 0.45 * (tc.BM * tc.BN) / 16384.0) / tc.eff;
      double t = 1.8 * rounds * (kper + 2) * tile_cost * (waste > 1.3 ? waste : 1.0);
      if (split > 1) t += 6.0 + 2.0 * (double)split * p.batch * p.M * p.N * 4 / 3.0e6;
      if (only >= 0 && force_split > 0 && split != force_split) continue;
      if (t < best_t - 1e-9) { best_t = t; best = GemmPlan{tc.id, split}; }
    }
  }
  return best;
}

int gemm_plan_split(const GemmArgs& p) { return gemm_plan(p).split; }

void launch_gemm(const GemmArgs& p, float* ws, hipStream_t s) {
  const bool mfma_ok = (p.K % 8 == 0) && (!p.conv || p.Cin % 8 == 0) &&
                       (p.conv || p.lda % 8 == 0) && (p.ldw % 8 == 0);
  if (launch_gemv(p, s)) return;
  if (!mfma_ok) {
    if (p.act == ACT_GEGLU || p.act == ACT_SWIGLU) return;
    long long total = (long long)p.M * p.N;
    dim3 grid((unsigned)((total + 255) / 256), 1, p.batch);
    if (p.conv)
      hipLaunchKernelGGL(gemm_simt_kernel<1>, grid, dim3(256), 0, s, p);
    else
      hipLaunchKernelGGL(gemm_simt_kernel<0>, grid, dim3(256), 0, s, p);
    return;
  }
  const bool buf = buf_ok(p);
  const GemmTile* t = gemm_tile(p.cfg);
  const GemmTileFamily fam = t != nullptr ? t->family : kTileStatic;
  if (fam == kTileAreg && gemm_areg_ok(p)) {
    launch_gemm_areg(p, s);
    return;
  }
  if (fam == kTilePingPong && family_runs(fam, p)) {
    if (!p.conv) gemm_pp_c0_launch(p, ws, s);
    else gemm_pp_c2_launch(p, ws, s);
    return;
  }
  if (!p.conv) {
    if (buf) gemm_c0_buf_launch(p, ws, s);
    else gemm_c0_launch(p, ws, s);
  } else if (p.Cin % 64 == 0) {
    if (p.upsample) gemm_c3_launch(p, ws, s);
    else if (buf) gemm_c2_buf_launch(p, ws, s);
    else gemm_c2_launch(p, ws, s);
  } else {
    gemm_c1_launch(p, ws, s);
  }
}
```

### cassmantle_amd/ops/csrc/gemm_impl.h

```cpp
#pragma once
#include <stdlib.h>

#include "common.h"
#include "gemm_tiles.h"
#include "kernels.h"

#ifndef GEMM_DIAG_APRO
#define GEMM_DIAG_APRO 0
#endif
#ifndef GEMM_FRAG_PREFETCH
#define GEMM_FRAG_PREFETCH 0
#endif

namespace {

__device__ uint4 g_zero_page[4];

constexpr int BK = 64;

CM_DEVICE int swz(int row, int chunk) { return chunk ^ ((row >> 1) & 7); }

#ifndef GEMM_PF_SELF
#define GEMM_PF_SELF 0
#endif
#ifndef GEMM_RASTER_G
#define GEMM_RASTER_G 4
#endif
CM_DEVICE void tile_of(int lin, int nM, int nN, int raster, int& tm, int& tn) {
  const int G = min(raster > 0 ? raster : GEMM_RASTER_G, nM);
  if (G > 1) {
    const int grp = lin / (G * nN);
    const int gs = min(G, nM - grp * G);
    const int r = lin - grp * G * nN;
    tm = grp * G + r % gs;
    tn = r / gs;
  } else {
    tn = lin % nN;
    tm = lin / nN;
  }
}

typedef __attribute__((address_space(3))) void lds_void;

CM_DEVICE void glds16(const void* src, uint4* lds_wave_base) {
  __builtin_amdgcn_global_load_lds(src, (lds_void*)lds_wave_base, 16, 0, 0);
}

CM_DEVICE void blds16(__amdgpu_buffer_rsrc_t rs, uint4* lds_wave_base, int voff, int soff) {
  __builtin_amdgcn_raw_ptr_buffer_load_lds(rs, (lds_void*)lds_wave_base, 16, voff, soff, 0, 0);
}

CM_DEVICE __amdgpu_buffer_rsrc_t make_rsrc(const void* base, long long bytes) {
  return __builtin_amdgcn_make_buffer_rsrc(const_cast<void*>(base), (short)0, (int)bytes, 0x00020000);
}

template <int N>
CM_DEVICE void wait_vmcnt() { asm volatile("s_waitcnt vmcnt(%0)" ::"n"(N) : "memory"); }

CM_DEVICE void add4(float* o, uint2 v) {
  o[0] += bf2f(v.x & 0xffff); o[1] += bf2f(v.x >> 16); o[2] += bf2f(v.y & 0xffff); o[3] += bf2f(v.y >> 16);
}

CM_DEVICE float2 ln_row(const GemmArgs& p, int m, double inv_k) {
  if (p.ln_rows_fx != nullptr) {
    const longlong2 v = reinterpret_cast<const longlong2*>(p.ln_rows_fx)[m];
    const double mean = (double)v.x * (inv_k * (1.0 / STAT_SCALE_SUM));
    const double var = fmax((double)v.y * (inv_k * (1.0 / STAT_SCALE_SQ)) - mean * mean, 0.0);
    return make_float2((float)mean, rsqrtf((float)var + p.ln_eps));
  }
  return reinterpret_cast<const float2*>(p.ln_rows)[m];
}
CM_DEVICE void ln_apply4(float2 ms, const float* __restrict__ wsum, float* o) {
#pragma unroll
  for (int r = 0; r < 4; ++r) o[r] = ms.y * fmaf(-ms.x, wsum[r], o[r]);
}
CM_DEVICE void ln_fold4(const GemmArgs& p, int m, int wn, float* o) {
  const float2 ms = ln_row(p, m, 1.0 / (double)p.K);
#pragma unroll
  for (int r = 0; r < 4; ++r) o[r] = ms.y * fmaf(-ms.x, p.ln_wsum[wn + r], o[r]);
}

CM_DEVICE long long out_row(const GemmArgs& p, int m, int z) {
  if (!p.parity) return m;
  const int hw = p.Ho * p.Wo;
  const int img = m / hw;
  const int r = m - img * hw;
  const int i = r / p.Wo, j = r - i * p.Wo;
  return ((long long)img * 2 * p.Ho + 2 * i + (z >> 1)) * (2 * p.Wo) + 2 * j + (z & 1);
}

template <bool OUTF32>
CM_DEVICE void epilogue4(const GemmArgs& p, int batch, int m, int n, float* o) {
  const int hw = p.Ho * p.Wo;
  const int bimg = (p.chan_bias != nullptr) ? (m / hw) : 0;
  const long long cbs = p.ldcb ? p.ldcb : p.N;
  const bool full = (n + 4 <= p.N) && (p.N % 4 == 0) && (p.ldc % 4 == 0) && (cbs % 4 == 0);
  const long long om = out_row(p, m, batch);
  if (p.ln_rows || p.ln_rows_fx) ln_fold4(p, m, n, o);
#pragma unroll
  for (int r = 0; r < 4; ++r) o[r] *= p.alpha;
  if (full) {
    if (p.bias) add4(o, *reinterpret_cast<const uint2*>(p.bias + n));
    if (p.chan_bias) add4(o, *reinterpret_cast<const uint2*>(p.chan_bias + (long long)bimg * cbs + n));
    if (p.act != ACT_NONE) {
#pragma unroll
      for (int r = 0; r < 4; ++r) o[r] = apply_act(o[r], p.act);
    }
    if (p.residual) add4(o, *reinterpret_cast<const uint2*>(p.residual + om * p.ldc + n));
    if (!OUTF32 && kv8_store4(p, m, n, o)) return;
    if constexpr (OUTF32) {
      float* C = reinterpret_cast<float*>(p.C) + (long long)batch * p.sC + om * p.ldc + n;
      *reinterpret_cast<float4*>(C) = make_float4(o[0], o[1], o[2], o[3]);
    } else {
      uint16_t* C = reinterpret_cast<uint16_t*>(p.C) + (long long)batch * p.sC + om * p.ldc + n;
      *reinterpret_cast<uint2*>(C) = make_uint2(pack2(o[0], o[1]), pack2(o[2], o[3]));
    }
  } else {
#pragma unroll
    for (int r = 0; r < 4; ++r) {
      if (n + r >= p.N) break;
      float v = o[r];
      if (p.bias) v += bf2f(p.bias[n + r]);
      if (p.chan_bias) v += bf2f(p.chan_bias[(long long)bimg * cbs + n + r]);
      v = apply_act(v, p.act);
      if (p.residual) v += bf2f(p.residual[om * p.ldc + n + r]);
      if constexpr (OUTF32)
        reinterpret_cast<float*>(p.C)[(long long)batch * p.sC + om * p.ldc + n + r] = v;
      else
        reinterpret_cast<uint16_t*>(p.C)[(long long)batch * p.sC + om * p.ldc + n + r] = f2bf(v);
    }
  }
}

template <bool OUTF32>
CM_DEVICE void epilogue4_call(const GemmArgs& p, int batch, int m, int n, f32x4_t v) {
  float o[4] = {v[0], v[1], v[2], v[3]};
  epilogue4<OUTF32>(p, batch, m, n, o);
}

CM_DEVICE void gated_epilogue4_call(const GemmArgs& p, int batch, int m, int n, f32x4_t hv, f32x4_t gv) {
  float o[4], hh[4] = {hv[0], hv[1], hv[2], hv[3]}, gg[4] = {gv[0], gv[1], gv[2], gv[3]};
  if (p.ln_rows || p.ln_rows_fx) { ln_fold4(p, m, n, hh); ln_fold4(p, m, p.N + n, gg); }
#pragma unroll
  for (int r = 0; r < 4; ++r) {
    float h = hh[r], g = gg[r];
    if (p.bias) { h += bf2f(p.bias[n + r]); g += bf2f(p.bias[p.N + n + r]); }
    o[r] = gate_f(h, g, p.act);
  }
  uint16_t* C = reinterpret_cast<uint16_t*>(p.C) + (long long)batch * p.sC + (long long)m * p.ldc + n;
  if (p.residual) add4(o, *reinterpret_cast<const uint2*>(p.residual + (long long)m * p.ldc + n));
  *reinterpret_cast<uint2*>(C) = make_uint2(pack2(o[0], o[1]), pack2(o[2], o[3]));
}

template <int BM, int BN, int WM, int WN, bool GEGLU, bool OUTF32, int TI, int TJ, int THREADS, bool SPLIT_DIRECT = false>
CM_DEVICE void tile_epilogue(const GemmArgs& p, f32x4_t (&acc)[TI][TJ], uint4* smem, float* __restrict__ partial,
                             int m0, int n0, int batch, int wm, int wn, int tid, int nsplit, int split_id,
                             bool has_acc = true) {
  const int lane = tid & 63;
  const int fr = lane & 15, fq = lane >> 4;
  if constexpr (!OUTF32) {
    constexpr int OBN = GEGLU ? BN / 2 : BN;
    constexpr int OST = OBN + 8;
    const long long cbs = p.ldcb ? p.ldcb : p.N;
    const bool lds_ok = nsplit == 1 && (p.N % 8 == 0) && (p.ldc % 8 == 0) && (cbs % 4 == 0);
    if (lds_ok) {
      __syncthreads();
      uint16_t* T = reinterpret_cast<uint16_t*>(smem);
      const int hw = p.Ho * p.Wo;
      const double inv_k = 1.0 / (double)p.K;
      if (has_acc) {
#pragma unroll
      for (int j = 0; j < TJ; ++j) {
        const int ml = wm * (BM / WM) + 16 * j + fr;
        const int m = m0 + ml;
        const int bimg = (p.chan_bias != nullptr && m < p.M) ? (m / hw) : 0;
        const bool lnf = (p.ln_rows != nullptr || p.ln_rows_fx != nullptr) && m < p.M;
        const float2 lnm = lnf ? ln_row(p, m, inv_k) : make_float2(0.f, 1.f);
        if constexpr (GEGLU) {
#pragma unroll
          for (int pi = 0; pi < TI / 2; ++pi) {
            const int nl = wn * (BN / WN / 2) + 16 * pi + 4 * fq;
            const int n = n0 + nl;
            float o[4], hh[4], gg[4];
#pragma unroll
            for (int r = 0; r < 4; ++r) { hh[r] = acc[2 * pi][j][r]; gg[r] = acc[2 * pi + 1][j][r]; }
            if (lnf && n < p.N) { ln_apply4(lnm, p.ln_wsum + n, hh); ln_apply4(lnm, p.ln_wsum + p.N + n, gg); }
#pragma unroll
            for (int r = 0; r < 4; ++r) {
              float h = hh[r], g = gg[r];
              if (p.bias && n < p.N) { h += bf2f(p.bias[n + r]); g += bf2f(p.bias[p.N + n + r]); }
              o[r] = gate_f(h, g, p.act);
            }
            *reinterpret_cast<uint2*>(T + ml * OST + nl) = make_uint2(pack2(o[0], o[1]), pack2(o[2], o[3]));
          }
        } else {
#pragma unroll
          for (int i = 0; i < TI; ++i) {
            const int nl = wn * (BN / WN) + 16 * i + 4 * fq;
            const int n = n0 + nl;
            float o[4] = {acc[i][j][0], acc[i][j][1], acc[i][j][2], acc[i][j][3]};
            if (lnf && n < p.N) ln_apply4(lnm, p.ln_wsum + n, o);
#pragma unroll
            for (int r = 0; r < 4; ++r) o[r] *= p.alpha;
            if (n < p.N && m < p.M) {
              if (p.bias) add4(o, *reinterpret_cast<const uint2*>(p.bias + n));
              if (p.chan_bias) add4(o, *reinterpret_cast<const uint2*>(p.chan_bias + (long long)bimg * cbs + n));
              if (p.act != ACT_NONE) {
#pragma unroll
                for (int r = 0; r < 4; ++r) o[r] = apply_act(o[r], p.act);
              }
            }
            *reinterpret_cast<uint2*>(T + ml * OST + nl) = make_uint2(pack2(o[0], o[1]), pack2(o[2], o[3]));
          }
        }
      }
      }
      __syncthreads();
      constexpr int CPR = OBN / 8;
      uint16_t* Cb = reinterpret_cast<uint16_t*>(p.C) + (long long)batch * p.sC;
      auto finish = [&](int row, int c8) -> uint4 {
        const int m = m0 + row, n = n0 + c8 * 8;
        const long long om = out_row(p, m, batch);
        uint4 v = *reinterpret_cast<const uint4*>(T + row * OST + c8 * 8);
        if (p.residual) {
          const uint4 rv = *reinterpret_cast<const uint4*>(p.residual + om * p.ldc + n);
          float a[8], b[8];
          unpack8(v, a);
          unpack8(rv, b);
#pragma unroll
          for (int e = 0; e < 8; ++e) a[e] += b[e];
          v = pack8(a);
        }
        if (p.kv8 != nullptr && n >= p.kv8_col0) {
          if (n < p.kv8_col0 + 64 * p.kv8_hk) {
            float a[8];
            unpack8(v, a);
            const int rel = n - p.kv8_col0, b = m / p.kv8_ntok, key = m - b * p.kv8_ntok;
            const long long bh = (long long)b * p.kv8_hk + (rel >> 6);
            *reinterpret_cast<uint2*>(p.kv8 + (bh * p.kv8_ntok + key) * 64 + (rel & 63)) =
                make_uint2(f8x4(a[0], a[1], a[2], a[3]), f8x4(a[4], a[5], a[6], a[7]));
          }
          return v;
        }
        *reinterpret_cast<uint4*>(Cb + om * p.ldc + n) = v;
        return v;
      };
      if (p.stats == nullptr) {
        for (int c = tid; c < BM * CPR; c += THREADS) {
          const int row = c / CPR, c8 = c - row * CPR;
          if (m0 + row >= p.M || n0 + c8 * 8 >= p.N) continue;
          const uint4 v = finish(row, c8);
          if (p.row_stats != nullptr) *reinterpret_cast<uint4*>(T + row * OST + c8 * 8) = v;
        }
        if (p.row_stats != nullptr) {
          __syncthreads();
          for (int row = tid; row < BM; row += THREADS) {
            const int m = m0 + row;
            if (m >= p.M) break;
            float sm = 0.f, sq = 0.f;
            for (int c8 = 0; c8 < CPR && n0 + c8 * 8 < p.N; ++c8) {
              float f[8];
// ... 469 lines not shown
  }
#endif

  if constexpr (STAGES == 2) {
    if (nk > 0) stage(kt0, 0);
    __syncthreads();
    for (int t = 0; t < nk; t += 2) {
      if (t + 1 < nk) stage(kt0 + t + 1, 1);
      compute(0);
      __syncthreads();
      if (t + 1 >= nk) break;
      if (t + 2 < nk) stage(kt0 + t + 2, 0);
      compute(1);
      __syncthreads();
    }
  } else {
    constexpr int S = STAGES;
    const int npt = w_last_round ? NPT : NPT - 1;
    auto wait_tiles = [&](int k) {
      if (npt == NPT) {
        if (k <= 0) wait_vmcnt<0>();
        else if (k == 1) wait_vmcnt<NPT>();
        else if (k == 2) wait_vmcnt<2 * NPT>();
        else wait_vmcnt<3 * NPT>();
      } else {
        if (k <= 0) wait_vmcnt<0>();
        else if (k == 1) wait_vmcnt<NPT - 1>();
        else if (k == 2) wait_vmcnt<2 * (NPT - 1)>();
        else wait_vmcnt<3 * (NPT - 1)>();
      }
    };
    if (dma_wave) {
#pragma unroll
      for (int s0 = 0; s0 < S - 1; ++s0)
        if (s0 < nk) stage(kt0 + s0, s0);
    }
    for (int t = 0; t < nk; ++t) {
      if (dma_wave) wait_tiles(min(S - 2, nk - 1 - t));
      asm volatile("s_waitcnt lgkmcnt(0)" ::: "memory");
      __builtin_amdgcn_s_barrier();
      if (dma_wave && t + S - 1 < nk) stage(kt0 + t + S - 1, (t + S - 1) % S);
      if (mma_wave) compute(t % S);
    }
  }

  tile_epilogue<BM, BN, WM, WN, GEGLU, OUTF32, TI, TJ, THREADS>(p, acc, smem, partial, m0, n0, batch, wm, wn, tid,
                                                               gridDim.y, blockIdx.y, mma_wave);
#if GEMM_PF_SELF
  asm volatile("" ::"v"(pf_acc));
#endif
}

template <bool OUTF32>
__global__ void splitk_reduce_kernel(GemmArgs p, const float* __restrict__ partial, int split) {
  const int bz = blockIdx.y;
  partial += (long long)bz * split * p.M * p.N;
  const long long nq = (long long)p.M * (p.N / 4);
  for (long long i = (long long)blockIdx.x * blockDim.x + threadIdx.x; i < nq; i += (long long)gridDim.x * blockDim.x) {
    const int m = (int)(i / (p.N / 4));
    const int n = (int)(i - (long long)m * (p.N / 4)) * 4;
    float o[4] = {0.f, 0.f, 0.f, 0.f};
    for (int s = 0; s < split; ++s) {
      const float4 v = *reinterpret_cast<const float4*>(partial + ((long long)s * p.M + m) * p.N + n);
      o[0] += v.x; o[1] += v.y; o[2] += v.z; o[3] += v.w;
    }
    epilogue4<OUTF32>(p, bz, m, n, o);
  }
}

constexpr int SK_RB = 64;
constexpr int SK_QB = 16;
constexpr int SK_RL = 256 / SK_QB;
template <bool OUTF32>
__global__ void __launch_bounds__(256) splitk_reduce_stats_kernel(GemmArgs p, const float* __restrict__ partial,
                                                                  int split, int rb) {
  __shared__ float red[2][SK_RL][SK_QB * 4];
  const int bz = blockIdx.z;
  partial += (long long)bz * split * p.M * p.N;
  const int qd = threadIdx.x % SK_QB, rl = threadIdx.x / SK_QB;
  const int n = (blockIdx.x * SK_QB + qd) * 4;
  const int m0 = blockIdx.y * rb;
  const int m1 = min(p.M, m0 + rb);
  const bool on = n < p.N;
  const int shw = p.stats_hw;
  const bool single = (m0 / shw) == ((m1 - 1) / shw);
  float s4[4] = {0.f, 0.f, 0.f, 0.f}, q4[4] = {0.f, 0.f, 0.f, 0.f};
  int cur = -1;
  auto flush = [&]() {
    if (cur < 0) return;
#pragma unroll
    for (int e = 0; e < 4; ++e) {
      stat_atomic_add(p.stats + ((long long)cur * p.N + n + e) * 2 + 0, 0, s4[e]);
      stat_atomic_add(p.stats + ((long long)cur * p.N + n + e) * 2 + 1, 1, q4[e]);
      s4[e] = 0.f;
      q4[e] = 0.f;
    }
  };
  if (on) {
    for (int m = m0 + rl; m < m1; m += SK_RL) {
      float o[4] = {0.f, 0.f, 0.f, 0.f};
      const float* src = partial + (long long)m * p.N + n;
      const long long slab = (long long)p.M * p.N;
      int sl = 0;
      for (; sl + 4 <= split; sl += 4) {
        const float4 v0 = *reinterpret_cast<const float4*>(src + (sl + 0) * slab);
        const float4 v1 = *reinterpret_cast<const float4*>(src + (sl + 1) * slab);
        const float4 v2 = *reinterpret_cast<const float4*>(src + (sl + 2) * slab);
        const float4 v3 = *reinterpret_cast<const float4*>(src + (sl + 3) * slab);
        o[0] += (v0.x + v1.x) + (v2.x + v3.x);
        o[1] += (v0.y + v1.y) + (v2.y + v3.y);
        o[2] += (v0.z + v1.z) + (v2.z + v3.z);
        o[3] += (v0.w + v1.w) + (v2.w + v3.w);
      }
      for (; sl < split; ++sl) {
        const float4 v = *reinterpret_cast<const float4*>(src + sl * slab);
        o[0] += v.x; o[1] += v.y; o[2] += v.z; o[3] += v.w;
      }
      epilogue4<OUTF32>(p, bz, m, n, o);
      if (!single) {
        const int img = m / shw;
        if (img != cur) { flush(); cur = img; }
      }
#pragma unroll
      for (int e = 0; e < 4; ++e) {
        const float f = OUTF32 ? o[e] : bf2f(f2bf(o[e]));
        s4[e] += f;
        q4[e] = fmaf(f, f, q4[e]);
      }
    }
  }
  if (!single) {
    flush();
    return;
  }
#pragma unroll
  for (int e = 0; e < 4; ++e) {
    red[0][rl][qd * 4 + e] = s4[e];
    red[1][rl][qd * 4 + e] = q4[e];
  }
  __syncthreads();
  const int img = m0 / shw;
  if (threadIdx.x < 2 * SK_QB * 4) {
    const int st = threadIdx.x / (SK_QB * 4), col = threadIdx.x % (SK_QB * 4);
    const int nn = blockIdx.x * SK_QB * 4 + col;
    if (nn < p.N) {
      float a = 0.f;
#pragma unroll
      for (int r = 0; r < SK_RL; ++r) a += red[st][r][col];
      stat_atomic_add(p.stats + ((long long)img * p.N + nn) * 2 + st, st, a);
    }
  }
}

template <bool OUTF32>
void launch_splitk_reduce(const GemmArgs& p, float* ws, int split, hipStream_t s) {
  if (p.stats != nullptr) {
    static const int adapt = [] { const char* e = getenv("CASSMANTLE_SK_ADAPT"); return e ? atoi(e) : 1; }();
    const long long cols = (p.N / 4 + SK_QB - 1) / SK_QB;
    int rb = SK_RB;
    while (adapt && rb > SK_RL && cols * ((p.M + rb - 1) / rb) * p.batch < 512) rb /= 2;
    dim3 g2((unsigned)cols, (unsigned)((p.M + rb - 1) / rb), (unsigned)p.batch);
    hipLaunchKernelGGL(splitk_reduce_stats_kernel<OUTF32>, g2, dim3(256), 0, s, p, ws, split, rb);
  } else {
    const long long nq = (long long)p.M * (p.N / 4);
    const long long nb = (nq + 255) / 256;
    const unsigned rb = (unsigned)(nb < 2048 ? nb : 2048);
    hipLaunchKernelGGL(splitk_reduce_kernel<OUTF32>, dim3(rb, (unsigned)p.batch), dim3(256), 0, s, p, ws, split);
  }
}

template <int BM, int BN, int WM, int WN, int CONV, bool GEGLU, bool OUTF32, int STAGES, bool BUF, int NP = 0>
void launch_t(const GemmArgs& p, float* ws, hipStream_t s) {
  const int nN = GEGLU ? (p.N + BN / 2 - 1) / (BN / 2) : (p.N + BN - 1) / BN;
  const int nM = (p.M + BM - 1) / BM;
  const int split = (ws != nullptr && p.split > 1) ? p.split : 1;
  dim3 grid(nN * nM, split, p.batch);
  constexpr size_t lds_stage = (size_t)STAGES * (BM + BN) * BK * 2;
  constexpr size_t lds_epi = (size_t)BM * ((GEGLU ? BN / 2 : BN) + 8) * 2;
  constexpr size_t lds = lds_stage > lds_epi ? lds_stage : lds_epi;
  auto* kfn = &gemm_kernel<BM, BN, WM, WN, CONV, GEGLU, OUTF32, STAGES, BUF, NP>;
  if constexpr (lds > 65536) {
    static const bool once = [&] {
      (void)hipFuncSetAttribute((const void*)kfn, hipFuncAttributeMaxDynamicSharedMemorySize, (int)lds);
      return true;
    }();
    (void)once;
  }
  hipLaunchKernelGGL(kfn, grid, dim3(64 * (WM * WN + NP)), lds, s, p, ws);
  if (split > 1) launch_splitk_reduce<OUTF32>(p, ws, split, s);
}

template <int I, int CONV, bool GEGLU, bool OUTF32, bool BUF>
bool launch_row(int cfg, const GemmArgs& p, float* ws, hipStream_t s) {
  constexpr GemmTile t = kGemmTiles[I];
  if constexpr ((t.family == kTileStatic || (t.family == kTileDeep && BUF && !OUTF32)) && (!GEGLU || t.gated())) {
    if (t.id != cfg) return false;
    launch_t<t.BM, t.BN, GEGLU ? t.GWM : t.WM, GEGLU ? t.GWN : t.WN, CONV, GEGLU, OUTF32, t.stages, BUF, t.producers>(p, ws, s);
    return true;
  }
  return false;
}

template <int CONV, bool GEGLU, bool OUTF32, bool BUF, int... I>
void launch_cfg(const GemmArgs& p, float* ws, hipStream_t s, std::integer_sequence<int, I...>) {
  if (!(launch_row<I, CONV, GEGLU, OUTF32, BUF>(p.cfg, p, ws, s) || ...))
    (void)(launch_row<I, CONV, GEGLU, OUTF32, BUF>(gemm_default_tile(kTileStatic, GEGLU), p, ws, s) || ...);
}

template <int CONV, bool BUF>
void launch_tiles(const GemmArgs& p, float* ws, hipStream_t s) {
  if (p.act == ACT_GEGLU || p.act == ACT_SWIGLU) launch_cfg<CONV, true, false, BUF>(p, ws, s, GemmTileRows{});
  else if (p.out_f32) launch_cfg<CONV, false, true, BUF>(p, ws, s, GemmTileRows{});
  else launch_cfg<CONV, false, false, BUF>(p, ws, s, GemmTileRows{});
}

}

#define GEMM_TU_ENTRY(NAME, CONV, BUF) \
  void NAME(const GemmArgs& p, float* ws, hipStream_t s) { launch_tiles<CONV, BUF>(p, ws, s); }
```

### cassmantle_amd/ops/csrc/kernels.h

```cpp
#pragma once
#include <hip/hip_runtime.h>
#include <stdint.h>

struct GemmArgs {
  const uint16_t* A = nullptr;
  const uint16_t* W = nullptr;
  const uint16_t* bias = nullptr;
  const uint16_t* residual = nullptr;
  const uint16_t* chan_bias = nullptr;
  int ldcb = 0;
  void* C = nullptr;
  int M = 0, N = 0, K = 0, Nw = 0;
  int lda = 0, ldc = 0, ldw = 0;
  long long sA = 0, sW = 0, sC = 0;
  int batch = 1;
  float alpha = 1.f;
  int act = 0;
  int out_f32 = 0;
  int split = 1;
  int cfg = 0;
  int raster = 0;
  int conv = 0, IH = 0, IW = 0, Cin = 0, Ho = 0, Wo = 0, stride = 1, pad = 0, ksize = 1, upsample = 0;
  int parity = 0;
  const uint16_t* rms_gamma = nullptr;
  float rms_eps = 0.f;
  const uint16_t* A2 = nullptr;
  int lda2 = 0, ka = 0;
  const float* ln_rows = nullptr;
  const float* ln_wsum = nullptr;
  float ln_eps = 0.f;
  const long long* ln_rows_fx = nullptr;
  long long* row_stats = nullptr;
  const long long* gn_stats = nullptr;
  const uint16_t* gn_gamma = nullptr;
  const uint16_t* gn_beta = nullptr;
  int gn_groups = 0, gn_hw = 0;
  float gn_eps = 0.f;
  long long* stats = nullptr;
  int stats_hw = 0;
  uint8_t* kv8 = nullptr;
  int kv8_col0 = 0, kv8_ntok = 0, kv8_hk = 0;
};
#define GEMM_MAX_SPLIT 16
struct GemmPlan { int cfg; int split; };
GemmPlan gemm_plan(const GemmArgs& p);
int gemm_plan_split(const GemmArgs& p);
void gemm_set_override(int cfg, int split);
#include <string>
std::string gemm_key(const GemmArgs& p);
void gemm_tune_set(const std::string& key, int cfg, int split);
void gemm_tune_clear();
int gemm_tune_size();
void gemm_record_keys(bool on);
std::string gemm_last_key();
void gemm_last_plan(int* cfg, int* split);
void launch_gemm(const GemmArgs& p, float* ws, hipStream_t s);

struct AttnArgs {
  const uint16_t* q; const uint16_t* k; const uint16_t* v; uint16_t* o;
  long long q_sb, q_sn, q_sh;
  long long k_sb, k_sn, k_sh;
  long long v_sb, v_sn, v_sh;
  long long o_sb, o_sn, o_sh;
  int B, H, Nq, Nk, d;
  float scale;
  int causal;
  const int* kv_lens;
  int group = 1;
};
void launch_attention(const AttnArgs& a, hipStream_t s);
long long attention_d512_workspace(const AttnArgs& a);
void launch_attention_d512(const AttnArgs& a, float* ws, hipStream_t s);
long long attention_fp8_workspace(const AttnArgs& a, int Hk);
void set_fp8_attn_variant(int v);
void set_attn_d40_variant(int v);
void launch_attention_fp8(const AttnArgs& a, int Hk, uint8_t* ws, hipStream_t s, bool packed = false);
void launch_attention_fp8_pack(const AttnArgs& a, int Hk, uint8_t* ws, hipStream_t s);

void launch_group_norm(const uint16_t* x, const uint16_t* gamma, const uint16_t* beta, uint16_t* y,
                       float* ws, int B, long long S, int C, int G, float eps, int silu, hipStream_t s);
void launch_group_norm_cs(const uint16_t* x, const uint16_t* x2, const long long* stats_a, int Ca, const long long* stats_b,
                          const uint16_t* gamma, const uint16_t* beta, uint16_t* y, int B, long long S, int C,
                          int G, float eps, int silu, hipStream_t s);
void launch_channel_stats(const uint16_t* x, long long* stats, int B, long long S, int C, hipStream_t s);
long long group_norm_workspace(int B, long long S, int C);
void launch_layer_norm(const uint16_t* x, const uint16_t* gamma, const uint16_t* beta, uint16_t* y,
                       long long rows, int D, float eps, hipStream_t s);
bool gemm_areg_ok(const GemmArgs& p);
void launch_gemm_areg(const GemmArgs& p, hipStream_t s);
void launch_row_stats(const uint16_t* x, float* stats, long long rows, int D, float eps, hipStream_t s);
void launch_embed_layer_norm(const uint16_t* word, const long long* ids, const uint16_t* pos, int seq,
                             const uint16_t* add, const uint16_t* gamma, const uint16_t* beta, uint16_t* y,
                             long long rows, int D, float eps, hipStream_t s);
void launch_rms_norm(const uint16_t* x, const uint16_t* gamma, uint16_t* y, long long rows, int D, float eps,
                     hipStream_t s);

bool launch_gemv(const GemmArgs& p, hipStream_t s);
struct RopeArgs {
  const uint16_t* qkv; long long ld;
  const int* pos0;
  uint16_t* q_out;
  uint16_t* k_cache; uint16_t* v_cache;
  int B, T, H, Hk, d, L;
  float log2_theta;
};
void launch_rope_kv(const RopeArgs& a, hipStream_t s);
struct DecodeArgs {
  const uint16_t* q; long long q_sb;
  const uint16_t* k_cache; const uint16_t* v_cache;
  const int* lens;
  uint16_t* o; long long o_sb;
  float* ws;
  int* tickets;
  int B, H, Hk, d, L;
  float scale;
};
int decode_splits(int B, int Hk, int L);
void launch_lm_sample(const void* logits, int logits_f32, int V, const float* noise, const float* eos_bias, int eos,
                      float temperature, int k, long long* step, long long* out, long long* tok, int* pos, int* lens,
                      hipStream_t s);
void launch_decode_attention(const DecodeArgs& a, int ns, hipStream_t s);

void launch_gather_cosine(const void* table, int table_f32, int D, const int* ia, const int* ib,
                          float* out, int n, hipStream_t s);
void launch_pair_cosine(const float* a, const float* b, int D, float* out, int n, hipStream_t s);
void launch_cosine_gemv(const void* table, int table_f32, int V, int D, const void* vec, int vec_f32,
                        float* out, hipStream_t s);
int cosine_topk_workspace(int V, int k);
void launch_cosine_topk(const void* table, int table_f32, int V, int D, const void* vec, int vec_f32, int k,
                        unsigned long long* ws, float* vals, long long* idx, hipStream_t s);
void launch_mean_pool_l2(const uint16_t* h, const int* lens, float* out, int B, int T, int D, hipStream_t s);

void launch_gaussian_blur(const void* img, int u8, int H, int W, int C, const float* w, int R,
                          float* tmp, void* out, hipStream_t s);
void launch_to_uint8(const uint16_t* x, uint8_t* out, long long n, hipStream_t s);
void launch_timestep_embedding(const float* t, void* out, int B, int dim, int flip, float shift, int out_bf16,
                               hipStream_t s);
void launch_gather_add(const uint16_t* table, const int* ids, const uint16_t* pos, int seq, int D, long long rows,
                       uint16_t* out, hipStream_t s);
void launch_concat2(const uint16_t* a, int Da, const void* b, int Db, int b_f32, long long rows, uint16_t* out,
                    hipStream_t s);
void launch_silu_bf16(uint16_t* x, long long n, hipStream_t s);
void launch_latent_init(const float* x0, float c_in0, float* x, float* xs, float* hist, int nhist, uint16_t* unet_in,
                        long long n, int cfg, int cin, int cstride, hipStream_t s);
void launch_copy(const void* src, void* dst, long long bytes, hipStream_t s);
void launch_finalize_latents(const float* x, uint16_t* z, long long n, uint8_t* finite, hipStream_t s);
void launch_latent_step(const uint16_t* eps, float* x, float* hist, float* xs, const float* coef, const int* step,
                        uint16_t* unet_in, long long n, int cfg, int cin, int cstride, const void* tab0, void* buf0,
                        long long row_bytes0, const void* tab1, void* buf1, long long row_bytes1, int rows,
                        hipStream_t s);
void launch_advance_step(int* step, hipStream_t s);
void launch_zero(void* p, long long bytes, hipStream_t s);
void launch_prefetch(const void* p, long long bytes, int blocks, void* sink, hipStream_t s);
void launch_softmax_rows(const float* S, uint16_t* P, int rows, int cols, int Nq, int causal,
                         const int* kv_lens, hipStream_t s);

struct JpegArgs {
  const uint8_t* img = nullptr;
  int B = 0, H = 0, W = 0;
  int nb = 0;
  int mx = 0, my = 0;
  int restart = 0, nint = 0;
  const int* qtab = nullptr;
  const int* huff = nullptr;
  int16_t* coef = nullptr;
  uint32_t* lens = nullptr;
  uint32_t* offs = nullptr;
  uint32_t* base = nullptr;
  const uint8_t* header = nullptr;
  int hdr_len = 0;
  uint8_t* out = nullptr;
  uint8_t* planes = nullptr;
  uint8_t* dec = nullptr;
};
void launch_jpeg_count(const JpegArgs& a, hipStream_t s);
void launch_jpeg_write(const JpegArgs& a, hipStream_t s);
void launch_jpeg_reconstruct(const JpegArgs& a, hipStream_t s);
struct JpegDecodeIn {
  const uint8_t* bytes = nullptr;
  uint32_t nbytes = 0;
  const uint32_t* intervals = nullptr;
  const uint32_t* tables = nullptr;
  unsigned long long* status = nullptr;
  long long zero_bytes = 0;
};
void launch_jpeg_entropy_decode(const JpegArgs& a, const JpegDecodeIn& d, hipStream_t s);
struct JpegSyncIn {
  const uint32_t* lane0 = nullptr;
  const uint32_t* groups = nullptr;
  int ngroups = 0;
  uint32_t cb = 0;
  uint32_t* words = nullptr;
};
void launch_jpeg_entropy_decode_chunked(const JpegArgs& a, const JpegDecodeIn& d, const JpegSyncIn& y, int threads,
                                        hipStream_t s);

int blur_pil_max_tiled_radius();
void launch_blur_pil_tiled(const uint8_t* img, int H, int W, const int* table, int n, int rmax, int nslots,
                           uint8_t* out, hipStream_t s);
void launch_blur_pil_general(const uint8_t* img, int H, int W, int r, uint32_t ww, uint32_t fw, uint8_t* s1,
                             uint8_t* s2, uint8_t* out, hipStream_t s);
```

Baseline: 7.668 images/s.

## Fuse GroupNorm+SiLU into split-K reduce for small-resolution ResNet conv1

```diff
diff --git a/cassmantle_amd/models/layers.py b/cassmantle_amd/models/layers.py
--- a/cassmantle_amd/models/layers.py
+++ b/cassmantle_amd/models/layers.py
@@ -114,7 +114,11 @@
         if self.pad_in > self.cin:
             self.padded_weight(self.pad_in)
 
-    def forward(self, x, residual=None, upsample=False, chan_bias=None, stats=None, out=None):
+    def forward(self, x, residual=None, upsample=False, chan_bias=None, stats=None, out=None, gn=None):
+        if gn is not None:
+            assert not upsample and x.shape[-1] == self.cin, "Conv2d: GroupNorm request on a plain conv only"
+            return ops.conv2d(x, self.weight, self.bias, self.stride, self.padding, residual=residual,
+                              chan_bias=chan_bias, stats=stats, out=out, gn=gn)
         if out is not None:
             w = self.padded_weight(x.shape[-1]) if x.shape[-1] > self.cin else self.weight
             return ops.conv2d(x, w, self.bias, self.stride, self.padding, residual=residual,
diff --git a/cassmantle_amd/models/unet.py b/cassmantle_amd/models/unet.py
--- a/cassmantle_amd/models/unet.py
+++ b/cassmantle_amd/models/unet.py
@@ -74,9 +74,17 @@
             tb = tb_all[:, self._tb_off:self._tb_off + self.time_emb_proj.fout]
         else:
             tb = self.time_emb_proj(temb_silu)
-        s1 = arena.take(B, cout) if arena is not None else None
-        h = self.conv1(h, chan_bias=tb, stats=s1)
-        h = self.norm2(h, silu=True, stats=s1)
+        hip = h.device.type == "cuda" and ops.get_mode() == "hip"
+        if _GN_REDUCE and (not hip or (arena is not None and arena.on and _gn_reduce_level(h))):
+            n2 = self.norm2
+            req = ops.GroupNormRequest(n2.weight, n2.bias, n2.groups, n2.eps, True, want_y=False,
+                                       scratch_stats=arena.take(B, cout) if hip else None)
+            self.conv1(h, chan_bias=tb, gn=req)
+            h = req.out
+        else:
+            s1 = arena.take(B, cout) if arena is not None else None
+            h = self.conv1(h, chan_bias=tb, stats=s1)
+            h = self.norm2(h, silu=True, stats=s1)
         if pair and self.conv_shortcut is None:
             sc = torch.cat(x, dim=-1)
         elif pair:
@@ -91,6 +99,12 @@
 _LN_FOLD = os.environ.get("CASSMANTLE_LN_FOLD", "1") == "1"
 _LN_ROWSTATS = os.environ.get("CASSMANTLE_LN_ROWSTATS", "1") == "1"
 _GN_FOLD = os.environ.get("CASSMANTLE_GN_FOLD", "1") == "1"
+_GN_REDUCE = os.environ.get("CASSMANTLE_GN_REDUCE", "1") == "1"
+_GN_REDUCE_MAX_HW = int(os.environ.get("CASSMANTLE_GN_REDUCE_MAX_HW", "64"))
+
+
+def _gn_reduce_level(h: torch.Tensor) -> bool:
+    return h.shape[1] * h.shape[2] <= _GN_REDUCE_MAX_HW
 _FF_ROWSTATS = os.environ.get("CASSMANTLE_FF_ROWSTATS", "1") == "1"
 
 
diff --git a/cassmantle_amd/ops/__init__.py b/cassmantle_amd/ops/__init__.py
--- a/cassmantle_amd/ops/__init__.py
+++ b/cassmantle_amd/ops/__init__.py
@@ -88,6 +88,7 @@
     if _RECORD is not None:
         call = lambda: fn(*args, **kw)
         call.fn, call.args, call.kw = fn, args, kw
+        call.gn_fused = fn in (ext().gemm, ext().conv2d) and bool(ext().gemm_last_gn_fused())
         _RECORD.append((ext().gemm_last_key(), call))
 
 
@@ -127,10 +128,37 @@
         channel_stats_ref(y, stats)
 
 
+class GroupNormRequest:
+
+    def __init__(self, gamma: torch.Tensor, beta: torch.Tensor, groups: int, eps: float, silu: bool = False,
+                 out: Optional[torch.Tensor] = None, want_y: bool = True,
+                 scratch_stats: Optional[torch.Tensor] = None):
+        self.gamma, self.beta, self.groups, self.eps, self.silu = gamma, beta, int(groups), float(eps), bool(silu)
+        self.out, self.want_y, self.scratch_stats = out, bool(want_y), scratch_stats
+        self.fused: Optional[bool] = None
+
+    def _kw(self, shape, like: torch.Tensor) -> dict:
+        if self.out is None:
+            self.out = torch.empty(shape, device=like.device, dtype=like.dtype)
+        else:
+            assert self.out.shape == tuple(shape) and self.out.is_contiguous(), "GroupNormRequest: bad out"
+        return dict(gno_gamma=self.gamma, gno_beta=self.beta, gno_out=self.out, gno_groups=self.groups,
+                    gno_eps=self.eps, gno_silu=int(self.silu), gno_want_y=self.want_y, gno_stats=self.scratch_stats)
+
+    def _ref(self, y: torch.Tensor) -> Optional[torch.Tensor]:
+        yn = group_norm(y, self.groups, self.gamma, self.beta, self.eps, self.silu)
+        self.out = yn if self.out is None else self.out.copy_(yn)
+        return y if self.want_y else None
+
+
+def gemm_last_gn_fused() -> bool:
+    return bool(ext().gemm_last_gn_fused())
+
+
 def linear(x: torch.Tensor, w: torch.Tensor, bias: Optional[torch.Tensor] = None,
            residual: Optional[torch.Tensor] = None, act: Optional[str] = None,
            stats: Optional[torch.Tensor] = None, out: Optional[torch.Tensor] = None,
-           row_stats: Optional[torch.Tensor] = None) -> torch.Tensor:
+           row_stats: Optional[torch.Tensor] = None, gn: Optional[GroupNormRequest] = None) -> torch.Tensor:
     if not _use_hip(x):
         if x.device.type == "cuda":
             y = _torch_linear(x, w, bias, residual, act)
@@ -138,24 +166,32 @@
             y = ref.linear(x, w, bias, residual, act)
         if stats is not None:
             channel_stats_ref(y, stats)
+        if gn is not None:
+            y = gn._ref(y)
+            if y is None:
+                return None
         return y if out is None else out.copy_(y)
     K = x.shape[-1]
     x2 = x.reshape(-1, K)
     if not x2.is_contiguous():
         x2 = x2.contiguous()
     N = w.shape[0] // 2 if act in ("geglu", "swiglu") else w.shape[0]
+    gkw = gn._kw((*x.shape[:-1], N), x) if gn is not None else {}
+    want_y = gn is None or gn.want_y
     if out is None:
-        out = torch.empty((x2.shape[0], N), device=x.device, dtype=x.dtype)
+        out = torch.empty((x2.shape[0], N), device=x.device, dtype=x.dtype) if want_y else gn.out
     else:
         assert out.is_contiguous() and out.dtype == x.dtype and out.numel() == x2.shape[0] * N, "linear: bad out"
     o2 = out.view(x2.shape[0], N)
     r2 = residual.reshape(-1, N) if residual is not None else None
-    hw = x2.shape[0] // x.shape[0] if stats is not None else 0
+    hw = x2.shape[0] // x.shape[0] if (stats is not None or gn is not None) else 0
     if row_stats is not None:
         _launch(ext().gemm, x2, w, bias, r2, o2, _ACT[act], stats, hw, row_stats=row_stats)
     else:
-        _launch(ext().gemm, x2, w, bias, r2, o2, _ACT[act], stats, hw)
-    return out.view(*x.shape[:-1], N)
+        _launch(ext().gemm, x2, w, bias, r2, o2, _ACT[act], stats, hw, **gkw)
+    if gn is not None:
+        gn.fused = gemm_last_gn_fused()
+    return out.view(*x.shape[:-1], N) if want_y else None
 
 
 def gn_linear(x: torch.Tensor, stats: torch.Tensor, gamma: torch.Tensor, beta: torch.Tensor, groups: int,
@@ -289,7 +325,7 @@
 def conv2d(x: torch.Tensor, w: torch.Tensor, bias: Optional[torch.Tensor] = None, stride: int = 1,
            padding: int = 1, residual: Optional[torch.Tensor] = None, upsample: bool = False,
            chan_bias: Optional[torch.Tensor] = None, stats: Optional[torch.Tensor] = None,
-           out: Optional[torch.Tensor] = None) -> torch.Tensor:
+           out: Optional[torch.Tensor] = None, gn: Optional[GroupNormRequest] = None) -> torch.Tensor:
     if not _use_hip(x):
         if x.device.type == "cuda":
             y = _torch_conv(x, w, bias, stride, padding, residual, upsample, chan_bias)
@@ -297,6 +333,10 @@
             y = ref.conv2d(x, w, bias, stride, padding, residual, upsample, chan_bias)
         if stats is not None:
             channel_stats_ref(y, stats)
+        if gn is not None:
+            y = gn._ref(y)
+            if y is None:
+                return None
         return y if out is None else out.copy_(y)
     B, H, W, Cin = x.shape
     Cout, kh, kw, _ = w.shape
@@ -308,12 +348,17 @@
     Hi, Wi = (2 * H, 2 * W) if upsample else (H, W)
     Ho = (Hi + 2 * padding - kh) // stride + 1
     Wo = (Wi + 2 * padding - kw) // stride + 1
+    gkw = gn._kw((B, Ho, Wo, Cout), x) if gn is not None else {}
+    want_y = gn is None or gn.want_y
     if out is None:
-        out = torch.empty((B, Ho, Wo, Cout), device=x.device, dtype=x.dtype)
+        out = torch.empty((B, Ho, Wo, Cout), device=x.device, dtype=x.dtype) if want_y else gn.out
     else:
         assert out.shape == (B, Ho, Wo, Cout) and out.dtype == x.dtype and out.is_contiguous(), "conv2d: bad out"
-    _launch(ext().conv2d, x.contiguous(), w, bias, residual, chan_bias, out, stride, padding, int(upsample), stats)
-    return out
+    _launch(ext().conv2d, x.contiguous(), w, bias, residual, chan_bias, out, stride, padding, int(upsample), stats,
+            **gkw)
+    if gn is not None:
+        gn.fused = gemm_last_gn_fused()
+    return out if want_y else None
 
 
 _UP2_ROWS = ([[1.0, 0.0, 0.0], [0.0, 1.0, 1.0]], [[1.0, 1.0, 0.0], [0.0, 0.0, 1.0]])
diff --git a/cassmantle_amd/ops/csrc/bindings.cpp b/cassmantle_amd/ops/csrc/bindings.cpp
--- a/cassmantle_amd/ops/csrc/bindings.cpp
+++ b/cassmantle_amd/ops/csrc/bindings.cpp
@@ -58,15 +58,91 @@
   g_raster[1].store((int)gated);
 }
 
-void run_gemm(GemmArgs& p, const at::Tensor& like) {
+struct GnRequest {
+  bool on = false;
+  const uint16_t* gamma = nullptr;
+  const uint16_t* beta = nullptr;
+  uint16_t* out = nullptr;
+  int groups = 0, silu = 0;
+  float eps = 0.f;
+  bool want_y = true;
+  long long* scratch_stats = nullptr;
+  long long scratch_numel = 0;
+};
+GnRequest gn_request(const c10::optional<at::Tensor>& gamma, const c10::optional<at::Tensor>& beta,
+                     const c10::optional<at::Tensor>& out, int64_t groups, double eps, int64_t silu, bool want_y,
+                     const c10::optional<at::Tensor>& scratch_stats, const at::Tensor& y) {
+  GnRequest r;
+  if (!out.has_value() || !out->defined()) return r;
+  TORCH_CHECK(gamma.has_value() && gamma->defined() && beta.has_value() && beta->defined() && groups > 0,
+              "GroupNorm request: gamma, beta and groups are required");
+  const int64_t N = y.size(-1);
+  CHECK_DEV(*out); CHECK_BF16(*out); CHECK_CONTIG(*out); CHECK_BF16(y);
+  TORCH_CHECK(out->numel() == y.numel() && out->size(-1) == N, "GroupNorm request: out must have the output's shape");
+  TORCH_CHECK(gamma->numel() == N && beta->numel() == N && N % groups == 0 && N % 8 == 0,
+              "GroupNorm request: gamma / beta of Cout channels, Cout a multiple of groups and of 8");
+  TORCH_CHECK(!want_y || out->data_ptr() != y.data_ptr(), "GroupNorm request: out aliases y");
+  r.on = true;
+  r.gamma = opt_bptr(gamma); r.beta = opt_bptr(beta); r.out = reinterpret_cast<uint16_t*>(out->data_ptr());
+  r.groups = (int)groups; r.eps = (float)eps; r.silu = (int)silu; r.want_y = want_y;
+  if (scratch_stats.has_value() && scratch_stats->defined()) {
+    CHECK_DEV(*scratch_stats); CHECK_CONTIG(*scratch_stats);
+    TORCH_CHECK(scratch_stats->scalar_type() == at::kLong, "GroupNorm request: scratch statistics must be int64");
+    r.scratch_stats = reinterpret_cast<long long*>(scratch_stats->data_ptr<int64_t>());
+    r.scratch_numel = scratch_stats->numel();
+  }
+  return r;
+}
+thread_local bool g_last_gn_fused = false;
+
+void run_gemm(GemmArgs& p, const at::Tensor& like, const GnRequest* gn = nullptr) {
   raster_from_env();
   p.raster = g_raster[(p.act == 4 || p.act == 6) ? 1 : 0].load(std::memory_order_relaxed);
   TORCH_CHECK(p.stats == nullptr || (p.N % 8 == 0 && p.ldc == p.N),
               "gemm/conv2d stats: the output channel count must be a multiple of 8 (GroupNorm consumers)");
-  const GemmPlan plan = gemm_plan(p);
+  const bool has_gn = gn != nullptr && gn->on;
+  GemmPlan plan;
+  if (has_gn && p.stats == nullptr) {
+    static long long plan_only;
+    GemmArgs q = p;
+    q.stats = &plan_only;
+    plan = gemm_plan(q);
+  } else {
+    plan = gemm_plan(p);
+  }
   p.cfg = plan.cfg;
   p.split = plan.split;
   if (p.kv8 != nullptr) p.split = 1;
+  g_last_gn_fused = false;
+  at::Tensor tmp_y, tmp_stats;
+  GnReduceArgs gnr;
+  struct Bound {
+    ~Bound() { gemm_gn_reduce_bind(nullptr); }
+  } bound;
+  if (has_gn) {
+    TORCH_CHECK(!p.out_f32 && p.ldc == p.N && p.stats_hw > 0 && p.M % p.stats_hw == 0,
+                "GroupNorm request: bf16 output in images of stats_hw rows");
+    if (gemm_gn_reduce_ok(p, gn->groups)) {
+      gnr.out = gn->out; gnr.gamma = gn->gamma; gnr.beta = gn->beta;
+      gnr.groups = gn->groups; gnr.silu = gn->silu; gnr.eps = gn->eps;
+      gemm_gn_reduce_bind(&gnr);
+      if (!gn->want_y) p.C = nullptr;
+      g_last_gn_fused = true;
+    } else {
+      if (!gn->want_y) {
+        tmp_y = at::empty({(long long)p.batch * p.M, p.N}, like.options().dtype(at::kBFloat16));
+        p.C = tmp_y.data_ptr();
+      }
+      if (p.stats == nullptr && gn->scratch_stats != nullptr) {
+        TORCH_CHECK(gn->scratch_numel == 2LL * (p.M / p.stats_hw) * p.N, "GroupNorm request: scratch statistics [images, N, 2]");
+        p.stats = gn->scratch_stats;
+      } else if (p.stats == nullptr) {
+        tmp_stats = at::zeros({p.M / p.stats_hw, p.N, 2}, like.options().dtype(at::kLong));
+        p.stats = reinterpret_cast<long long*>(tmp_stats.data_ptr<int64_t>());
+      }
+    }
+  }
+  long long* const y_stats = p.stats;
   long long* post_stats = nullptr;
   if (p.stats != nullptr && (p.out_f32 || p.M <= 8 || (p.batch != 1 && !p.parity) || p.act == 4 || p.act == 6)) {
     post_stats = p.stats;
@@ -81,6 +157,9 @@
   if (post_stats != nullptr)
     launch_channel_stats(reinterpret_cast<const uint16_t*>(p.C), post_stats, p.M / p.stats_hw, p.stats_hw, p.N,
                          cur_stream());
+  if (has_gn && !g_last_gn_fused)
+    launch_group_norm_cs(reinterpret_cast<const uint16_t*>(p.C), nullptr, y_stats, p.N, nullptr, gn->gamma, gn->beta,
+                         gn->out, p.M / p.stats_hw, p.stats_hw, p.N, gn->groups, gn->eps, gn->silu, cur_stream());
 }
 
 void gemm(const at::Tensor& x, const at::Tensor& w, const c10::optional<at::Tensor>& bias,
@@ -90,8 +169,18 @@
           const c10::optional<at::Tensor>& kv8, int64_t kv8_col0, int64_t kv8_ntok, int64_t kv8_hk,
           const c10::optional<at::Tensor>& ln_rows_fx, const c10::optional<at::Tensor>& row_stats,
           const c10::optional<at::Tensor>& gn_stats, const c10::optional<at::Tensor>& gn_gamma,
-          const c10::optional<at::Tensor>& gn_beta, int64_t gn_groups, int64_t gn_hw, double gn_eps) {
+          const c10::optional<at::Tensor>& gn_beta, int64_t gn_groups, int64_t gn_hw, double gn_eps,
+          const c10::optional<at::Tensor>& gno_gamma, const c10::optional<at::Tensor>& gno_beta,
+          const c10::optional<at::Tensor>& gno_out, int64_t gno_groups, double gno_eps, int64_t gno_silu,
+          bool gno_want_y, const c10::optional<at::Tensor>& gno_stats) {
   CHECK_DEV(x); CHECK_BF16(x); CHECK_BF16(w); CHECK_CONTIG(w); CHECK_CONTIG(out);
+  const GnRequest gnq = gn_request(gno_gamma, gno_beta, gno_out, gno_groups, gno_eps, gno_silu, gno_want_y, gno_stats, out);
+  if (gnq.on)
+    TORCH_CHECK(stats_hw > 0 && !(gn_stats.has_value() && gn_stats->defined()) &&
+                    !(ln_rows_fx.has_value() && ln_rows_fx->defined()) && !(ln_wsum.has_value() && ln_wsum->defined()) &&
+                    !(row_stats.has_value() && row_stats->defined()) && !(kv8.has_value() && kv8->defined()),
+                "gemm: a GroupNorm request needs stats_hw and excludes the LayerNorm / GroupNorm input folds, "
+                "row statistics and kv8");
   TORCH_CHECK(x.dim() == 2 && w.dim() == 2 && out.dim() == 2, "gemm: 2-D operands expected");
   TORCH_CHECK(x.stride(1) == 1, "gemm: x rows must be contiguous");
   GemmArgs p;
@@ -127,6 +216,7 @@
     p.stats_hw = (int)stats_hw;
     p.stats = opt_stats(stats, p.M / stats_hw, p.N);
   }
+  if (gnq.on) p.stats_hw = (int)stats_hw;
   if (gn_stats.has_value() && gn_stats->defined()) {
     TORCH_CHECK(gn_gamma.has_value() && gn_beta.has_value() && gn_groups > 0 && gn_hw > 0 && p.M % gn_hw == 0,
                 "gemm: gn_stats needs gamma, beta, groups and rows per image");
@@ -203,7 +293,7 @@
       return;
     }
   }
-  run_gemm(p, out);
+  run_gemm(p, out, &gnq);
 }
 
 void row_stats(const at::Tensor& x, at::Tensor& out, double eps) {
@@ -261,8 +351,12 @@
 
 void conv2d(const at::Tensor& x, const at::Tensor& w, const c10::optional<at::Tensor>& bias,
             const c10::optional<at::Tensor>& residual, const c10::optional<at::Tensor>& chan_bias, at::Tensor& out,
-            int64_t stride, int64_t pad, int64_t upsample, const c10::optional<at::Tensor>& stats) {
+            int64_t stride, int64_t pad, int64_t upsample, const c10::optional<at::Tensor>& stats,
+            const c10::optional<at::Tensor>& gno_gamma, const c10::optional<at::Tensor>& gno_beta,
+            const c10::optional<at::Tensor>& gno_out, int64_t gno_groups, double gno_eps, int64_t gno_silu,
+            bool gno_want_y, const c10::optional<at::Tensor>& gno_stats) {
   CHECK_DEV(x); CHECK_BF16(x); CHECK_CONTIG(x); CHECK_BF16(w); CHECK_CONTIG(w); CHECK_CONTIG(out); CHECK_BF16(out);
+  const GnRequest gnq = gn_request(gno_gamma, gno_beta, gno_out, gno_groups, gno_eps, gno_silu, gno_want_y, gno_stats, out);
   TORCH_CHECK(x.dim() == 4 && w.dim() == 4 && out.dim() == 4, "conv2d: NHWC 4-D tensors expected");
   GemmArgs p;
   p.conv = 1;
@@ -290,7 +384,7 @@
   p.C = out.data_ptr();
   p.stats_hw = p.Ho * p.Wo;
   p.stats = opt_stats(stats, x.size(0), p.N);
-  run_gemm(p, out);
+  run_gemm(p, out, &gnq);
 }
 
 void conv2d_up2(const at::Tensor& x, const at::Tensor& w4, const c10::optional<at::Tensor>& bias,
@@ -1012,7 +1106,10 @@
         py::arg("ln_wsum") = py::none(), py::arg("ln_eps") = 0.0, py::arg("kv8") = py::none(),
         py::arg("kv8_col0") = 0, py::arg("kv8_ntok") = 0, py::arg("kv8_hk") = 0, py::arg("ln_rows_fx") = py::none(),
         py::arg("row_stats") = py::none(), py::arg("gn_stats") = py::none(), py::arg("gn_gamma") = py::none(),
-        py::arg("gn_beta") = py::none(), py::arg("gn_groups") = 0, py::arg("gn_hw") = 0, py::arg("gn_eps") = 0.0, nogil());
+        py::arg("gn_beta") = py::none(), py::arg("gn_groups") = 0, py::arg("gn_hw") = 0, py::arg("gn_eps") = 0.0,
+        py::arg("gno_gamma") = py::none(), py::arg("gno_beta") = py::none(), py::arg("gno_out") = py::none(),
+        py::arg("gno_groups") = 0, py::arg("gno_eps") = 0.0, py::arg("gno_silu") = 0, py::arg("gno_want_y") = true,
+        py::arg("gno_stats") = py::none(), nogil());
   m.def("row_stats", &row_stats, nogil());
   m.def("gemm_cat", &gemm_cat, nogil());
   m.def("group_norm_cat", &group_norm_cat, nogil());
@@ -1031,8 +1128,14 @@
   m.def("gemm_record_keys", [](bool on) { gemm_record_keys(on); });
   m.def("gemm_last_key", []() { return gemm_last_key(); });
   m.def("gemm_last_plan", []() { int c, sp; gemm_last_plan(&c, &sp); return std::vector<int64_t>{c, sp}; });
+  m.def("gemm_last_gn_fused", []() { return g_last_gn_fused; });
+  m.def("gemm_gn_reduce_set_gb", [](int64_t gb) { gemm_gn_reduce_set_gb((int)gb); });
   m.def("gemm_rms", &gemm_rms, nogil());
-  m.def("conv2d", &conv2d, nogil());
+  m.def("conv2d", &conv2d, py::arg("x"), py::arg("w"), py::arg("bias"), py::arg("residual"), py::arg("chan_bias"),
+        py::arg("out"), py::arg("stride"), py::arg("pad"), py::arg("upsample"), py::arg("stats"),
+        py::arg("gno_gamma") = py::none(), py::arg("gno_beta") = py::none(), py::arg("gno_out") = py::none(),
+        py::arg("gno_groups") = 0, py::arg("gno_eps") = 0.0, py::arg("gno_silu") = 0, py::arg("gno_want_y") = true,
+        py::arg("gno_stats") = py::none(), nogil());
   m.def("conv2d_up2", &conv2d_up2, nogil());
   m.def("bmm_nt", &bmm_nt, nogil());
   m.def("group_norm", &group_norm, nogil());
diff --git a/cassmantle_amd/ops/csrc/gemm.hip b/cassmantle_amd/ops/csrc/gemm.hip
--- a/cassmantle_amd/ops/csrc/gemm.hip
+++ b/cassmantle_amd/ops/csrc/gemm.hip
@@ -224,6 +224,27 @@
 
 int gemm_plan_split(const GemmArgs& p) { return gemm_plan(p).split; }
 
+static std::atomic<int> g_gnr_gb{0};
+static thread_local const GnReduceArgs* g_gnr_bound = nullptr;
+void gemm_gn_reduce_bind(const GnReduceArgs* g) { g_gnr_bound = g; }
+const GnReduceArgs* gemm_gn_reduce_bound() { return g_gnr_bound; }
+void gemm_gn_reduce_set_gb(int gb) { g_gnr_gb = gb; }
+int gemm_gn_reduce_gb() { return g_gnr_gb.load(std::memory_order_relaxed); }
+bool gemm_gn_reduce_ok(const GemmArgs& p, int groups) {
+  if (p.split <= 1 || p.batch != 1 || p.parity || p.out_f32 || is_gated(p.act) || p.kv8 != nullptr) return false;
+  const bool mfma_ok = (p.K % 8 == 0) && (!p.conv || p.Cin % 8 == 0) && (p.conv || p.lda % 8 == 0) && (p.ldw % 8 == 0);
+  if (p.M <= 8 || !mfma_ok) return false;
+  const GemmTile* t = gemm_tile(p.cfg);
+  if (t != nullptr && t->family == kTileAreg && gemm_areg_ok(p)) return false;
+  if (groups <= 0 || p.N % groups != 0) return false;
+  const int cg = p.N / groups;
+  if (cg % 4 != 0 || cg > 256) return false;
+  if (p.ldc != p.N || (p.ldcb ? p.ldcb : p.N) % 4 != 0) return false;
+  if (p.stats_hw <= 0 || p.M % p.stats_hw != 0) return false;
+  if (p.residual != nullptr && p.residual == p.C) return false;
+  return true;
+}
+
 void launch_gemm(const GemmArgs& p, float* ws, hipStream_t s) {
   const bool mfma_ok = (p.K % 8 == 0) && (!p.conv || p.Cin % 8 == 0) &&
                        (p.conv || p.lda % 8 == 0) && (p.ldw % 8 == 0);
diff --git a/cassmantle_amd/ops/csrc/gemm_impl.h b/cassmantle_amd/ops/csrc/gemm_impl.h
--- a/cassmantle_amd/ops/csrc/gemm_impl.h
+++ b/cassmantle_amd/ops/csrc/gemm_impl.h
@@ -89,7 +89,7 @@
   return ((long long)img * 2 * p.Ho + 2 * i + (z >> 1)) * (2 * p.Wo) + 2 * j + (z & 1);
 }
 
-template <bool OUTF32>
+template <bool OUTF32, bool STORE = true>
 CM_DEVICE void epilogue4(const GemmArgs& p, int batch, int m, int n, float* o) {
   const int hw = p.Ho * p.Wo;
   const int bimg = (p.chan_bias != nullptr) ? (m / hw) : 0;
@@ -107,6 +107,7 @@
       for (int r = 0; r < 4; ++r) o[r] = apply_act(o[r], p.act);
     }
     if (p.residual) add4(o, *reinterpret_cast<const uint2*>(p.residual + om * p.ldc + n));
+    if constexpr (!STORE) return;
     if (!OUTF32 && kv8_store4(p, m, n, o)) return;
     if constexpr (OUTF32) {
       float* C = reinterpret_cast<float*>(p.C) + (long long)batch * p.sC + om * p.ldc + n;
@@ -882,8 +883,15 @@
   }
 }
 
+
 template <bool OUTF32>
 void launch_splitk_reduce(const GemmArgs& p, float* ws, int split, hipStream_t s) {
+  if constexpr (!OUTF32) {
+    if (const GnReduceArgs* gq = gemm_gn_reduce_bound()) {
+      launch_splitk_reduce_gn(p, *gq, ws, split, s);
+      return;
+    }
+  }
   if (p.stats != nullptr) {
     static const int adapt = [] { const char* e = getenv("CASSMANTLE_SK_ADAPT"); return e ? atoi(e) : 1; }();
     const long long cols = (p.N / 4 + SK_QB - 1) / SK_QB;
diff --git a/cassmantle_amd/ops/csrc/gemm_reduce_gn.hip b/cassmantle_amd/ops/csrc/gemm_reduce_gn.hip
--- /dev/null
+++ b/cassmantle_amd/ops/csrc/gemm_reduce_gn.hip
@@ -0,0 +1,187 @@
+#include <stdlib.h>
+
+#include "gemm_impl.h"
+
+namespace {
+
+constexpr int GNR_U = 4;
+constexpr int GNR_KEEP = 24;
+constexpr int GNR_MAXW = 256;
+template <int NR, int THREADS>
+__global__ void __launch_bounds__(THREADS) splitk_reduce_gn_kernel(GemmArgs p, GnReduceArgs gq, const float* __restrict__ partial,
+                                                                   int split, int gb) {
+  static_assert(NR % GNR_U == 0 && NR <= GNR_KEEP, "kept rows: whole load groups, within the register budget");
+  __shared__ float sh[2 * 4 * THREADS + 2 * GNR_MAXW + 8];
+  float* red = sh;
+  float* tot = sh + 2 * 4 * THREADS;
+  float* gst = tot + 2 * GNR_MAXW;
+  const int tid = threadIdx.x;
+  const int Cg = p.N / gq.groups, W = gb * Cg, Q = W / 4, R = THREADS / Q;
+  const int qd = tid % Q, rl = tid / Q;
+  const bool act = rl < R;
+  const int S = p.stats_hw, img = blockIdx.y;
+  const int c0 = blockIdx.x * W;
+  const int n = c0 + qd * 4;
+  const int m0 = img * S;
+  const long long slab = (long long)p.M * p.N;
+  const bool store_y = p.C != nullptr;
+  const float* src0 = partial + (long long)m0 * p.N + n;
+  const uint2 gv = *reinterpret_cast<const uint2*>(gq.gamma + n);
+  const uint2 bv = *reinterpret_cast<const uint2*>(gq.beta + n);
+
+  auto sum_rows = [&](int r0, float (&o)[GNR_U][4]) {
+    const float* src[GNR_U];
+#pragma unroll
+    for (int u = 0; u < GNR_U; ++u) {
+      src[u] = src0 + (long long)min(r0 + u * R, S - 1) * p.N;
+      o[u][0] = 0.f; o[u][1] = 0.f; o[u][2] = 0.f; o[u][3] = 0.f;
+    }
+    int sl = 0;
+    for (; sl + 4 <= split; sl += 4) {
+      float4 v[GNR_U][4];
+#pragma unroll
+      for (int u = 0; u < GNR_U; ++u)
+#pragma unroll
+        for (int j = 0; j < 4; ++j) v[u][j] = *reinterpret_cast<const float4*>(src[u] + (sl + j) * slab);
+#pragma unroll
+      for (int u = 0; u < GNR_U; ++u) {
+        o[u][0] += (v[u][0].x + v[u][1].x) + (v[u][2].x + v[u][3].x);
+        o[u][1] += (v[u][0].y + v[u][1].y) + (v[u][2].y + v[u][3].y);
+        o[u][2] += (v[u][0].z + v[u][1].z) + (v[u][2].z + v[u][3].z);
+        o[u][3] += (v[u][0].w + v[u][1].w) + (v[u][2].w + v[u][3].w);
+      }
+    }
+    for (; sl < split; ++sl) {
+      float4 v[GNR_U];
+#pragma unroll
+      for (int u = 0; u < GNR_U; ++u) v[u] = *reinterpret_cast<const float4*>(src[u] + sl * slab);
+#pragma unroll
+      for (int u = 0; u < GNR_U; ++u) { o[u][0] += v[u].x; o[u][1] += v[u].y; o[u][2] += v[u].z; o[u][3] += v[u].w; }
+    }
+  };
+  auto finish = [&](int r, float* o, bool store) -> uint2 {
+    if (store) epilogue4<false, true>(p, 0, m0 + r, n, o);
+    else epilogue4<false, false>(p, 0, m0 + r, n, o);
+    return make_uint2(pack2(o[0], o[1]), pack2(o[2], o[3]));
+  };
+  auto unpack4 = [](uint2 w, float* f) {
+    f[0] = __uint_as_float(w.x << 16); f[1] = __uint_as_float(w.x & 0xffff0000u);
+    f[2] = __uint_as_float(w.y << 16); f[3] = __uint_as_float(w.y & 0xffff0000u);
+  };
+
+  uint2 keep[NR > 0 ? NR : 1];
+  float s4[4] = {0.f, 0.f, 0.f, 0.f}, q4[4] = {0.f, 0.f, 0.f, 0.f};
+  auto pass1_group = [&](int r0, uint2* kp) {
+    float o[GNR_U][4];
+    sum_rows(r0, o);
+#pragma unroll
+    for (int u = 0; u < GNR_U; ++u) {
+      if (r0 + u * R >= S) continue;
+      const uint2 w = finish(r0 + u * R, o[u], store_y);
+      float f[4];
+      unpack4(w, f);
+#pragma unroll
+      for (int e = 0; e < 4; ++e) { s4[e] += f[e]; q4[e] = fmaf(f[e], f[e], q4[e]); }
+      if (kp != nullptr) kp[u] = w;
+    }
+  };
+  if (act) {
+    if constexpr (NR > 0) {
+#pragma unroll
+      for (int k = 0; k < NR; k += GNR_U)
+        if (rl + k * R < S) pass1_group(rl + k * R, &keep[k]);
+    } else {
+      for (int r0 = rl; r0 < S; r0 += GNR_U * R) pass1_group(r0, nullptr);
+    }
+#pragma unroll
+    for (int e = 0; e < 4; ++e) {
+      red[rl * W + qd * 4 + e] = s4[e];
+      red[(R + rl) * W + qd * 4 + e] = q4[e];
+    }
+  }
+  __syncthreads();
+  for (int c = tid; c < 2 * W; c += THREADS) {
+    const int st = c / W, col = c - st * W;
+    float a = 0.f;
+    for (int r = 0; r < R; ++r) a += red[(st * R + r) * W + col];
+    tot[c] = a;
+    if (p.stats != nullptr) stat_atomic_add(p.stats + ((long long)img * p.N + c0 + col) * 2 + st, st, a);
+  }
+  __syncthreads();
+  if (tid < gb) {
+    long long si = 0, qi = 0;
+    for (int c = 0; c < Cg; ++c) {
+      si += __double2ll_rn((double)tot[tid * Cg + c] * STAT_SCALE_SUM);
+      qi += __double2ll_rn((double)tot[W + tid * Cg + c] * STAT_SCALE_SQ);
+    }
+    const double sm = stat_decode(si, 0), q = stat_decode(qi, 1);
+    const double cnt = (double)S * Cg;
+    const double mean = sm / cnt;
+    double var = q / cnt - mean * mean;
+    if (var < 0) var = 0;
+    gst[2 * tid] = (float)mean;
+    gst[2 * tid + 1] = (float)(1.0 / sqrt(var + (double)gq.eps));
+  }
+  __syncthreads();
+  if (!act) return;
+  float sc[4], sf[4];
+  {
+    float ga[4], be[4];
+    unpack4(gv, ga);
+    unpack4(bv, be);
+    const int g = (qd * 4) / Cg;
+#pragma unroll
+    for (int e = 0; e < 4; ++e) {
+      sc[e] = ga[e] * gst[2 * g + 1];
+      sf[e] = be[e] - gst[2 * g] * sc[e];
+    }
+  }
+  const int silu = gq.silu;
+  auto emit = [&](int r, uint2 w) {
+    float f[4];
+    unpack4(w, f);
+#pragma unroll
+    for (int e = 0; e < 4; ++e) {
+      const float o = fmaf(f[e], sc[e], sf[e]);
+      f[e] = silu ? silu_f(o) : o;
+    }
+    *reinterpret_cast<uint2*>(gq.out + (long long)(m0 + r) * p.N + n) = make_uint2(pack2(f[0], f[1]), pack2(f[2], f[3]));
+  };
+  if constexpr (NR > 0) {
+#pragma unroll
+    for (int k = 0; k < NR; ++k)
+      if (rl + k * R < S) emit(rl + k * R, keep[k]);
+  } else {
+    for (int r0 = rl; r0 < S; r0 += GNR_U * R) {
+      float o[GNR_U][4];
+      sum_rows(r0, o);
+#pragma unroll
+      for (int u = 0; u < GNR_U; ++u)
+        if (r0 + u * R < S) emit(r0 + u * R, finish(r0 + u * R, o[u], false));
+    }
+  }
+}
+
+int gnr_pick_gb(const GemmArgs& p, const GnReduceArgs& gq) {
+  int gb = gemm_gn_reduce_gb() & 7;
+  if (gb <= 0) gb = 1;
+  const int Cg = p.N / gq.groups;
+  while (gb > 1 && (gq.groups % gb != 0 || gb * Cg > GNR_MAXW)) gb /= 2;
+  return gb;
+}
+
+}
+
+void launch_splitk_reduce_gn(const GemmArgs& p, const GnReduceArgs& gq, float* ws, int split, hipStream_t s) {
+  const int gb = gnr_pick_gb(p, gq);
+  const int Q = gb * (p.N / gq.groups) / 4;
+  const int rpt = (p.stats_hw + 256 / Q - 1) / (256 / Q);
+  const int rpt_wide = (p.stats_hw + 1024 / Q - 1) / (1024 / Q);
+  const bool wide = rpt > GNR_U && rpt_wide <= GNR_U && !(gemm_gn_reduce_gb() & 16);
+  const dim3 g((unsigned)(gq.groups / gb), (unsigned)(p.M / p.stats_hw));
+  if (wide) hipLaunchKernelGGL((splitk_reduce_gn_kernel<4, 1024>), g, dim3(1024), 0, s, p, gq, ws, split, gb);
+  else if (rpt <= 4) hipLaunchKernelGGL((splitk_reduce_gn_kernel<4, 256>), g, dim3(256), 0, s, p, gq, ws, split, gb);
+  else if (rpt <= 12) hipLaunchKernelGGL((splitk_reduce_gn_kernel<12, 256>), g, dim3(256), 0, s, p, gq, ws, split, gb);
+  else if (rpt <= GNR_KEEP) hipLaunchKernelGGL((splitk_reduce_gn_kernel<GNR_KEEP, 256>), g, dim3(256), 0, s, p, gq, ws, split, gb);
+  else hipLaunchKernelGGL((splitk_reduce_gn_kernel<0, 256>), g, dim3(256), 0, s, p, gq, ws, split, gb);
+}
diff --git a/cassmantle_amd/ops/csrc/kernels.h b/cassmantle_amd/ops/csrc/kernels.h
--- a/cassmantle_amd/ops/csrc/kernels.h
+++ b/cassmantle_amd/ops/csrc/kernels.h
@@ -54,6 +54,19 @@
 void gemm_record_keys(bool on);
 std::string gemm_last_key();
 void gemm_last_plan(int* cfg, int* split);
+struct GnReduceArgs {
+  uint16_t* out = nullptr;
+  const uint16_t* gamma = nullptr;
+  const uint16_t* beta = nullptr;
+  int groups = 0, silu = 0;
+  float eps = 0.f;
+};
+void gemm_gn_reduce_bind(const GnReduceArgs* g);
+const GnReduceArgs* gemm_gn_reduce_bound();
+bool gemm_gn_reduce_ok(const GemmArgs& p, int groups);
+void launch_splitk_reduce_gn(const GemmArgs& p, const GnReduceArgs& g, float* ws, int split, hipStream_t s);
+void gemm_gn_reduce_set_gb(int gb);
+int gemm_gn_reduce_gb();
 void launch_gemm(const GemmArgs& p, float* ws, hipStream_t s);
 
 struct AttnArgs {
```

After: 7.657 images/s. About the same (-0.1%).
